# houzhijian/CONE

Measured on AMD Instinct MI355X. Metric: windows/sec + queries/sec, Ego4D-NLQ win_len=90 d=256 top-k=20, higher is better.
Workload: dtype f32

## Files before the change

### cone_amd/_lib.py

```python
from __future__ import annotations

import ctypes as C
import os

HERE = os.path.dirname(os.path.abspath(__file__))
LIB_PATH = os.path.join(HERE, "libcone_hip.so")

MAX_LAYERS = 8
MAX_PROJ = 3

c_float_p = C.c_void_p


class Linear(C.Structure):
    _fields_ = [("w", C.c_void_p), ("b", C.c_void_p)]


class LNorm(C.Structure):
    _fields_ = [("g", C.c_void_p), ("b", C.c_void_p)]


class Mha(C.Structure):
    _fields_ = [("in_proj_w", C.c_void_p), ("in_proj_b", C.c_void_p), ("out_proj", Linear)]

# ... 140 lines not shown
    "cone_criterion_forward": (C.c_int, [C.c_void_p, C.c_void_p, C.c_void_p, C.c_void_p, C.c_void_p, C.c_void_p, C.c_int,
                                         C.c_void_p, C.c_void_p, C.c_int, C.c_void_p, C.c_int, C.c_int, C.c_int,
                                         C.c_float, C.c_float, C.c_float, C.c_float, C.c_float, C.c_void_p, C.c_void_p,
                                         C.c_void_p, C.c_void_p]),
    "cone_adapter_nce": (C.c_int, [C.c_void_p, C.c_int, C.c_float, C.c_void_p, C.c_void_p]),
    "cone_prof_enable": (C.c_int, [C.c_int]),
    "cone_prof_collect": (C.c_int64, [C.c_void_p, C.c_int64]),
    "cone_eval_recall": (C.c_int, [C.c_void_p, C.c_void_p, C.c_void_p, C.c_int, C.c_int, C.c_void_p, C.c_int,
                                   C.c_void_p, C.c_int, C.c_int, C.c_void_p, C.c_void_p, C.c_void_p]),
    "cone_eval_window_recall": (C.c_int, [C.c_void_p, C.c_int, C.c_int, C.c_void_p, C.c_double, C.c_int, C.c_void_p,
                                          C.c_int, C.c_void_p, C.c_void_p]),
    "cone_model_set_option": (C.c_int, [C.c_void_p, C.c_char_p, C.c_int]),
    "cone_model_get_dims": (C.c_int, [C.c_void_p, C.POINTER(ModelDims)]),
    "cone_session_arena_bytes": (C.c_size_t, [C.c_void_p, C.c_int64, C.c_int]),
    "cone_session_workspace": (C.c_size_t, [C.c_void_p, C.c_int64, C.c_int]),
    "cone_session_index": (C.c_int, [C.c_void_p, C.c_void_p, C.c_int64, C.c_int, C.c_void_p, C.c_size_t, C.c_void_p, C.c_size_t,
                                     C.POINTER(Session), C.c_void_p]),
    "cone_session_query_layout": (C.c_int, [C.POINTER(C.c_int32), C.c_int, C.c_int, C.c_int64, C.c_int, C.c_int, C.c_int]
                                  + [C.c_void_p] * 8 + [C.c_void_p]),
    "cone_session_localize_workspace": (C.c_size_t, [C.c_void_p, C.POINTER(Session), C.POINTER(C.c_int32), C.c_int, C.c_int,
                                                     C.c_int, C.POINTER(SessionParams)]),
    "cone_session_localize": (C.c_int, [C.c_void_p, C.POINTER(Session), C.c_void_p, C.POINTER(C.c_int32), C.c_int, C.c_void_p,
                                        C.c_int, C.c_int, C.POINTER(SessionParams), C.c_void_p, C.c_void_p, C.c_void_p,
                                        C.c_void_p, C.c_size_t, C.c_void_p]),
    "cone_library_arena_bytes": (C.c_size_t, [C.c_void_p, C.c_int64, C.c_int]),
    "cone_library_open": (C.c_int, [C.c_void_p, C.c_int64, C.c_int, C.c_void_p, C.c_size_t, C.POINTER(Library)]),
    "cone_library_add_workspace": (C.c_size_t, [C.c_void_p, C.c_int64]),
    "cone_library_add": (C.c_int, [C.c_void_p, C.POINTER(Library), C.c_int64, C.c_void_p, C.c_int64, C.c_void_p, C.c_size_t,
                                   C.c_void_p]),
    "cone_library_query_layout": (C.c_int, [C.POINTER(C.c_int32)] * 3 + [C.c_int] * 5 + [C.c_void_p] * 8 + [C.c_void_p]),
    "cone_library_localize_workspace": (C.c_size_t, [C.c_void_p, C.POINTER(Library)] + [C.POINTER(C.c_int32)] * 3
                                        + [C.c_int, C.c_int, C.POINTER(SessionParams)]),
    "cone_library_localize": (C.c_int, [C.c_void_p, C.POINTER(Library), C.POINTER(C.c_int32), C.POINTER(C.c_int32), C.c_void_p,
                                        C.POINTER(C.c_int32), C.c_int, C.c_void_p, C.c_int, C.POINTER(SessionParams), C.c_void_p,
                                        C.c_void_p, C.c_void_p, C.c_size_t, C.c_void_p]),
    "cone_library_scan_workspace": (C.c_size_t, [C.POINTER(Library), C.c_int64, C.c_int64, C.c_int, C.c_int, C.c_int]),
    "cone_library_scan": (C.c_int, [C.c_void_p, C.POINTER(Library)] + [C.c_void_p] * 3 + [C.c_int64, C.c_int64, C.c_void_p, C.c_int,
                                    C.c_int, C.c_int, C.POINTER(SessionParams)] + [C.c_void_p] * 4 + [C.c_void_p, C.c_size_t,
                                                                                                    C.c_void_p]),
    "cone_library_localize_ranked_workspace": (C.c_size_t, [C.c_void_p, C.POINTER(Library)] + [C.POINTER(C.c_int32)] * 3
                                               + [C.c_int, C.c_int, C.POINTER(SessionParams)]),
    "cone_library_localize_ranked": (C.c_int, [C.c_void_p, C.POINTER(Library), C.POINTER(C.c_int32), C.POINTER(C.c_int32), C.c_void_p,
                                               C.POINTER(C.c_int32), C.c_int, C.c_void_p, C.c_int, C.POINTER(SessionParams),
                                               C.POINTER(C.c_int32), C.POINTER(C.c_int32), C.c_void_p, C.c_void_p, C.c_int, C.c_int64,
                                               C.c_int, C.c_void_p, C.c_void_p, C.c_void_p, C.c_size_t, C.c_void_p]),
    "cone_library_move_stage_bytes": (C.c_size_t, [C.POINTER(Library), C.c_int64]),
    "cone_library_move_rows": (C.c_int, [C.c_void_p, C.POINTER(Library), C.POINTER(Library)] + [C.c_void_p] * 3 + [C.c_int64] * 4
                               + [C.c_void_p, C.c_size_t, C.c_void_p]),
    "cone_library_budget_workspace": (C.c_size_t, [C.c_int, C.c_int64, C.c_int, C.c_int]),
    "cone_library_budget": (C.c_int, [C.c_void_p, C.c_int, C.c_int64, C.c_int, C.c_int] + [C.c_void_p] * 4
                            + [C.c_void_p, C.c_size_t, C.c_void_p]),
    "cone_library_localize_ragged_workspace": (C.c_size_t, [C.c_void_p, C.POINTER(Library)] + [C.POINTER(C.c_int32)] * 3
                                               + [C.c_int, C.POINTER(C.c_int32), C.POINTER(SessionParams), C.c_int]),
    "cone_library_localize_ragged": (C.c_int, [C.c_void_p, C.POINTER(Library), C.POINTER(C.c_int32), C.POINTER(C.c_int32), C.c_void_p,
                                               C.POINTER(C.c_int32), C.c_int, C.c_void_p, C.POINTER(C.c_int32),
                                               C.POINTER(SessionParams), C.POINTER(C.c_int32), C.POINTER(C.c_int32), C.c_void_p,
                                               C.c_void_p, C.c_int, C.c_int64, C.c_int, C.c_void_p, C.c_void_p, C.c_void_p, C.c_size_t,
                                               C.c_void_p]),
    "cone_corpus_fuse_nms": (C.c_int, [C.c_void_p] * 5 + [C.c_int, C.c_int, C.c_double, C.c_int, C.c_int] + [C.c_void_p] * 4),
    "cone_library_localize_candidates_workspace": (C.c_size_t, [C.c_void_p, C.POINTER(Library)] + [C.POINTER(C.c_int32)] * 3
                                                   + [C.c_int, C.POINTER(C.c_int32), C.POINTER(SessionParams), C.c_int]),
    "cone_library_localize_candidates": (C.c_int, [C.c_void_p, C.POINTER(Library), C.POINTER(C.c_int32), C.POINTER(C.c_int32),
                                                   C.c_void_p, C.POINTER(C.c_int32), C.c_int, C.c_void_p, C.POINTER(C.c_int32),
                                                   C.POINTER(SessionParams), C.POINTER(C.c_int32), C.POINTER(C.c_int32), C.c_void_p,
                                                   C.c_void_p, C.c_int, C.c_int64, C.c_int, C.c_void_p, C.c_void_p, C.c_size_t,
                                                   C.c_void_p]),
    "cone_watch_plan": (C.c_int, [C.c_void_p, C.c_void_p, C.c_int, C.c_int, C.c_void_p] + [C.c_int] * 4 + [C.c_void_p] * 8),
    "cone_watch_store": (C.c_int, [C.c_void_p] * 3 + [C.c_int] * 5 + [C.c_void_p] * 3),
    "cone_watch_pool_plan": (C.c_int, [C.c_void_p] * 9 + [C.c_int] * 7 + [C.c_void_p] * 8),
    "cone_watch_pool_store": (C.c_int, [C.c_void_p, C.c_void_p, C.c_int] + [C.c_void_p] * 4 + [C.c_int] * 5 + [C.c_void_p] * 3),
    "cone_library_shadow_bytes": (C.c_size_t, [C.POINTER(Library)]),
    "cone_library_shadow_open": (C.c_int, [C.POINTER(Library), C.c_void_p, C.c_size_t, C.POINTER(LibraryShadow)]),
    "cone_library_shadow_index": (C.c_int, [C.c_void_p, C.POINTER(Library), C.POINTER(LibraryShadow), C.c_int64, C.c_int64, C.c_void_p]),
    "cone_library_scan_certified_workspace": (C.c_size_t, [C.POINTER(Library), C.c_int64, C.c_int64, C.c_int64] + [C.c_int] * 4),
    "cone_library_scan_certified": (C.c_int, [C.c_void_p, C.POINTER(Library), C.POINTER(LibraryShadow)] + [C.c_void_p] * 4
                                    + [C.c_int64] * 3 + [C.c_void_p] + [C.c_int] * 4 + [C.POINTER(SessionParams)] + [C.c_void_p] * 3
                                    + [C.c_void_p, C.c_size_t, C.c_void_p]),
    "cone_test_gemm": (C.c_int, [C.c_void_p, C.c_void_p, C.c_int, C.c_void_p, C.c_void_p, C.c_void_p,
                                 C.c_void_p, C.c_void_p, C.c_void_p, C.c_void_p, C.c_void_p, C.c_int, C.c_int,
                                 C.c_int, C.c_int, C.c_void_p]),
    "cone_test_gemm_tall": (C.c_int, [C.c_void_p, C.c_void_p, C.c_int, C.c_void_p, C.c_void_p, C.c_void_p,
                                      C.c_void_p, C.c_void_p, C.c_void_p, C.c_void_p, C.c_void_p, C.c_int, C.c_int,
                                      C.c_int, C.c_int, C.c_int, C.c_int, C.c_void_p, C.c_int, C.c_void_p]),
    "cone_test_gemm_bf16_image_bytes": (C.c_size_t, [C.c_int, C.c_int]),
    "cone_test_gemm_bf16": (C.c_int, [C.c_void_p, C.c_void_p, C.c_int, C.c_void_p, C.c_void_p, C.c_void_p,
                                      C.c_void_p, C.c_void_p, C.c_void_p, C.c_void_p, C.c_void_p, C.c_int, C.c_int,
                                      C.c_int, C.c_int, C.c_void_p, C.c_int, C.c_int, C.c_void_p, C.c_void_p]),
    "cone_test_ffn": (C.c_int, [C.c_void_p] * 8 + [C.c_int, C.c_int, C.c_void_p]),
    "cone_test_proj_ffn": (C.c_int, [C.c_void_p] * 13 + [C.c_int, C.c_int, C.c_void_p]),
    "cone_test_tail_form": (C.c_int, [C.c_void_p] * 13 + [C.c_int, C.c_int] + [C.c_void_p] * 3 + [C.c_int, C.c_void_p, C.c_int, C.c_int,
                                                                               C.c_void_p, C.c_void_p]),
    "cone_test_proj_ffn_spread_scratch_bytes": (C.c_size_t, [C.c_int]),
    "cone_test_proj_ffn_spread": (C.c_int, [C.c_void_p] * 13 + [C.c_int, C.c_int, C.c_void_p, C.c_void_p]),
    "cone_test_ffn_split_image_bytes": (C.c_size_t, [C.c_int]),
    "cone_test_ffn_split": (C.c_int, [C.c_void_p] * 8 + [C.c_int, C.c_int, C.c_void_p, C.c_int, C.c_void_p]),
    "cone_test_rows_split_image_bytes": (C.c_size_t, [C.c_int]),
    "cone_test_rows_split": (C.c_int, [C.c_void_p] * 4 + [C.c_int, C.c_int, C.c_void_p, C.c_int, C.c_void_p]),
    "cone_test_proj_split_image_bytes": (C.c_size_t, []),
    "cone_test_proj_ffn_split": (C.c_int, [C.c_void_p] * 13 + [C.c_int, C.c_int, C.c_void_p, C.c_void_p, C.c_int, C.c_void_p]),
    "cone_test_enc_attn": (C.c_int, [C.c_int] + [C.c_void_p] * 9 + [C.c_int, C.c_int, C.c_int, C.c_void_p]),
    "cone_test_dec_cross": (C.c_int, [C.c_void_p] * 9 + [C.c_int] * 4 + [C.c_void_p, C.c_void_p]),
    "cone_test_dec_cross_slab_floats": (C.c_size_t, []),
    "cone_test_enc_attn_txt": (C.c_int, [C.c_int] + [C.c_void_p] * 10 + [C.c_int, C.c_int, C.c_int, C.c_void_p]),
    "cone_test_small_attn": (C.c_int, [C.c_void_p, C.c_int, C.c_void_p, C.c_int, C.c_void_p, C.c_int, C.c_void_p, C.c_int,
                                       C.c_void_p, C.c_int, C.c_int, C.c_int, C.c_void_p]),
    "cone_test_dec_cross_ex": (C.c_int, [C.c_void_p] * 10 + [C.c_int] * 4 + [C.c_void_p] * 4 + [C.c_int, C.c_void_p]),
    "cone_test_layernorm": (C.c_int, [C.c_void_p, C.c_void_p, C.c_void_p, C.c_void_p, C.c_int64, C.c_int,
                                      C.c_void_p]),
    "cone_test_gen_attn": (C.c_int, [C.c_void_p, C.c_int, C.c_void_p, C.c_int, C.c_void_p, C.c_int, C.c_void_p, C.c_int,
                                     C.c_void_p, C.c_void_p] + [C.c_int] * 5 + [C.c_void_p]),
    "cone_test_grid_limit_y": (C.c_int, []),
    "cone_test_scan_lengths": (C.c_int, [C.c_void_p, C.c_void_p, C.c_int, C.c_void_p, C.c_void_p]),
    "cone_test_compact_index": (C.c_int, [C.c_void_p, C.c_void_p, C.c_int, C.c_void_p, C.c_void_p, C.c_void_p, C.c_int,
                                          C.c_void_p, C.c_int, C.c_void_p]),
    "cone_test_pack_pos": (C.c_int, [C.c_void_p] * 11 + [C.c_int, C.c_int] + [C.c_void_p] * 4),
    "cone_test_gen_pack_pos": (C.c_int, [C.c_void_p] * 10 + [C.c_int] * 3 + [C.c_void_p] * 4),
    "cone_test_pack_l0": (C.c_int, [C.c_void_p] * 15 + [C.c_int, C.c_int, C.c_void_p]),
    "cone_test_row_index": (C.c_int, [C.c_void_p] * 6 + [C.c_int, C.c_int, C.c_void_p]),
    "cone_test_add_pos_rows": (C.c_int, [C.c_void_p] * 5 + [C.c_int, C.c_int] + [C.c_void_p] * 3),
    "cone_test_txt_pos_rows": (C.c_int, [C.c_void_p] * 3 + [C.c_int, C.c_int] + [C.c_void_p] * 3 + [C.c_int] + [C.c_void_p] * 3),
    "cone_test_gen_txt_pos_rows": (C.c_int, [C.c_void_p] * 3 + [C.c_int, C.c_int] + [C.c_void_p] * 3 + [C.c_int, C.c_void_p, C.c_int,
                                                                                                    C.c_void_p, C.c_void_p]),
    "cone_test_saliency": (C.c_int, [C.c_void_p] * 7 + [C.c_int, C.c_void_p, C.c_int, C.c_int, C.c_void_p]),
    "cone_test_gen_saliency": (C.c_int, [C.c_void_p] * 7 + [C.c_int, C.c_void_p, C.c_int, C.c_int, C.c_int, C.c_void_p]),
    "cone_test_rowdot": (C.c_int, [C.c_void_p, C.c_int, C.c_void_p, C.c_void_p, C.c_void_p, C.c_int, C.c_int64, C.c_int, C.c_int,
                                   C.c_void_p]),
    "cone_test_gen_rowdot": (C.c_int, [C.c_void_p, C.c_int, C.c_void_p, C.c_void_p, C.c_void_p, C.c_int, C.c_int64, C.c_int, C.c_int,
                                       C.c_int, C.c_void_p]),
    "cone_test_tile_rows": (C.c_int, [C.c_void_p, C.c_int, C.c_int64, C.c_void_p]),
    "cone_test_tile_rows2": (C.c_int, [C.c_void_p] * 4 + [C.c_int, C.c_int64, C.c_void_p]),
}
EXPORTS = tuple(_SIGNATURES)

_lib = None


class ConeHipError(RuntimeError):
    pass


def load():
    global _lib
    if _lib is not None:
        return _lib
    if not os.path.exists(LIB_PATH):
        raise ConeHipError(
            f"{LIB_PATH} is missing: build the HIP extension with `python -m cone_amd.build` "
            "(hipcc, gfx950). cone_amd has no CPU fallback.")
    import torch
    lib = C.CDLL(LIB_PATH)
    for name, (res, args) in _SIGNATURES.items():
        fn = getattr(lib, name)
        fn.restype = res
        fn.argtypes = args
    if lib.cone_abi_version() != 8:
        raise ConeHipError("libcone_hip.so ABI version mismatch; rebuild")
    _lib = lib
    return lib


_pylists = None


def pylists():
    global _pylists
    if _pylists is None:
# ... 42 lines not shown
```

### cone_amd/build.py

```python
from __future__ import annotations

import os
import subprocess
import sys
from concurrent.futures import ThreadPoolExecutor

HERE = os.path.dirname(os.path.abspath(__file__))
CSRC = os.path.join(HERE, "csrc")
OBJ = os.path.join(CSRC, "_obj")
LIB = os.path.join(HERE, "libcone_hip.so")
PYLISTS = os.path.join(HERE, "_cone_pylists.so")
SOURCES = ["api.hip", "gemm.hip", "rowops.hip", "attention.hip", "window_ops.hip", "prefilter.hip",
           "postproc.hip", "prof.hip", "dec_cross.hip", "metrics.hip", "ffn.hip", "criterion.hip", "dec_cross_mfma.hip", "ffn_split.hip", "ffn_wide.hip",
           "general.hip", "ffn_bf16.hip", "gemm_bf16.hip", "gemm_tall.hip", "session.hip", "library_move.hip",
           "library_budget.hip", "library_corpus.hip", "library_watch.hip", "library_watch_pool.hip"]
FLAGS = ["-O3", "--offload-arch=gfx950", "-fPIC", "-std=c++17", "-Wall", "-Wno-unused-function"]
NO_CONTRACT = {"window_ops.hip", "postproc.hip", "metrics.hip", "criterion.hip", "general.hip", "library_corpus.hip"}


def _deps_mtime():
    hdrs = [os.path.join(CSRC, f) for f in os.listdir(CSRC) if f.endswith(".h")]
    hdrs += [os.path.join(HERE, "..", "include", "cone_hip.h"), __file__]
    return max(os.path.getmtime(h) for h in hdrs)


def _compile(src):
    obj = os.path.join(OBJ, src.replace(".hip", ".o"))
    stamp = obj + ".flags"
    path = os.path.join(CSRC, src)
    extra = ["-ffp-contract=off"] if src in NO_CONTRACT else []
    extra += os.environ.get("CONE_HIPCC_FLAGS", "").split()
    flags = " ".join([*FLAGS, *extra])
    try:
        with open(stamp) as f:
            same_flags = f.read() == flags
    except OSError:
        same_flags = False
    if same_flags and os.path.exists(obj) and os.path.getmtime(obj) >= max(os.path.getmtime(path), _deps_mtime()):
        return obj
    cmd = ["hipcc", *FLAGS, *extra, "-c", path, "-o", obj]
    r = subprocess.run(cmd, capture_output=True, text=True)
    if r.returncode != 0:
        raise RuntimeError(f"hipcc failed for {src}:\n{r.stdout}\n{r.stderr}")
    with open(stamp, "w") as f:
        f.write(flags)
    if r.stderr.strip():
        sys.stderr.write(r.stderr)
    return obj


def build(force: bool = False) -> str:
    os.makedirs(OBJ, exist_ok=True)
    if force:
        for f in os.listdir(OBJ):
            os.remove(os.path.join(OBJ, f))
    with ThreadPoolExecutor(max_workers=4) as ex:
        objs = list(ex.map(_compile, SOURCES))
    if (not os.path.exists(LIB)) or any(os.path.getmtime(o) > os.path.getmtime(LIB) for o in objs):
        r = subprocess.run(["hipcc", "--offload-arch=gfx950", "-shared", "-fPIC", "-o", LIB, *objs],
                           capture_output=True, text=True)
        if r.returncode != 0:
            raise RuntimeError(f"link failed:\n{r.stdout}\n{r.stderr}")
    try:
        build_pylists()
    except (RuntimeError, OSError) as e:
        try:
            if os.path.exists(PYLISTS) and os.path.getmtime(PYLISTS) < os.path.getmtime(os.path.join(CSRC, "pylists.c")):
                os.remove(PYLISTS)
        except OSError:
            pass
        sys.stderr.write(f"cone_amd.build: _cone_pylists.so not built ({str(e).splitlines()[0]}); "
                         "submission lists will be built by the Python loop\n")
    return LIB


def build_pylists() -> str:
    import sysconfig
    src = os.path.join(CSRC, "pylists.c")
    if os.path.exists(PYLISTS) and os.path.getmtime(PYLISTS) >= max(os.path.getmtime(src), os.path.getmtime(__file__)):
        return PYLISTS
    r = subprocess.run(["gcc", "-O2", "-shared", "-fPIC", "-Wall", "-I", sysconfig.get_paths()["include"], src, "-o", PYLISTS],
                       capture_output=True, text=True)
    if r.returncode != 0:
        raise RuntimeError(f"gcc failed for pylists.c:\n{r.stdout}\n{r.stderr}")
    return PYLISTS


if __name__ == "__main__":
    print(build(force="--force" in sys.argv))
```

### cone_amd/csrc/api.hip

```cpp
#include <stdarg.h>
#include <string.h>

#include <vector>

#include "common.h"
#include "gemm_tall.h"
#include "rows_chain.h"

namespace cone {

static thread_local char g_err[512] = "";
void set_error(const char* fmt, ...) {
    va_list ap;
    va_start(ap, fmt);
    vsnprintf(g_err, sizeof(g_err), fmt, ap);
    va_end(ap);
}

struct Linear { const float* w = nullptr; const float* b = nullptr; };
struct LNorm { const float* g = nullptr; const float* b = nullptr; };
struct Mha { const float* in_w = nullptr; const float* in_b = nullptr; Linear out; };
struct EncLayer { Mha sa; Linear l1, l2; LNorm n1, n2; };
struct DecLayer { Mha sa, ca; Linear l1, l2; LNorm n1, n2, n3; };

}

struct cone_model {
    int d, heads, ff, n_enc, n_dec, nq, n_proj, dt, dv, dvm, has_adapter;
    float* arena = nullptr;
    cone::LNorm vproj_ln[CONE_MAX_PROJ], tproj_ln[CONE_MAX_PROJ];
    cone::Linear vproj[CONE_MAX_PROJ], tproj[CONE_MAX_PROJ];
    cone::EncLayer enc[CONE_MAX_LAYERS];
    cone::DecLayer dec[CONE_MAX_LAYERS];
    cone::LNorm dec_norm;
    const float* query_embed = nullptr;
    cone::Linear class_embed, span[3], saliency, adapter[2];
    const float* dim_t = nullptr;
    const float* txt_pos_emb = nullptr; int txt_pos_rows = 0; cone::LNorm txt_pos_ln;
    int pre_norm = 0; cone::LNorm enc_norm;
    cone::Linear dec_k, dec_v;
    const float* dec_vT[CONE_MAX_LAYERS] = {};
    float* dec0_tgt1 = nullptr; float* dec0_dq = nullptr; float* dec0_scratch = nullptr;
    float* dec_sa_tab[CONE_MAX_LAYERS] = {}; float* dec_ca_tab[CONE_MAX_LAYERS] = {};
    float* tab_arena = nullptr; const float* tab_pos_rows = nullptr; const float* tab_pos_qk = nullptr; int tab_max_v_l = 0;
    int opt_dec_fold = 2;
    int opt_dec0_const = 1;
    int opt_l0_gather = 1;
    int opt_pos_tables = 1;
    int opt_gemm = 0;
    int opt_gemm_tall_min = -1;
    cone::TailWeights enc_tail[CONE_MAX_LAYERS] = {}, dec_tail[CONE_MAX_LAYERS] = {};
    char* split_img = nullptr; char* bf16_img = nullptr;
    int opt_qkv_fused = 1;
    int opt_split_bf16 = 0;
    int opt_bf16 = 0;
    int opt_res_gather = 1;
    int opt_spread = 1;
    int opt_chain = 1;
    int opt_ffn_fused = 2;
    int gen_native = 0;
    int opt_general = 0;
    int opt_general_bf16 = 0;
    char* gen_bf16_img = nullptr;
    struct GenImage { const float* W; const void* img; };
    std::vector<GenImage> gen_bf16_images;
    int opt_max_tokens = CONE_MAX_WINDOW_TOKENS;
    bool long_windows() const { return opt_max_tokens > CONE_MAX_WINDOW_TOKENS; }
    bool general() const { return gen_native || opt_general || long_windows(); }
};

namespace cone {

struct ArenaBuilder {
    struct Item { const float* src; size_t n; const float** dst; };
    std::vector<Item> items;
    size_t total = 0;
    void add(const float* src, size_t n, const float** dst) {
        items.push_back({src, n, dst});
        total += align_up(n, 64);
    }
};

static int dec0_constants(cone_model* m, hipStream_t s);
static int build_pos_tables(const cone_model* m, int max_v_l, float* pos_rows, float* pos_qk, hipStream_t s);
static int64_t pos_table_rows(int max_v_l) { return (int64_t)max_v_l * (max_v_l + 1) / 2 + 1; }

static void free_model(cone_model* m) {
    if (m->arena) (void)hipFree(m->arena);
    if (m->split_img) (void)hipFree(m->split_img);
    if (m->bf16_img) (void)hipFree(m->bf16_img);
    if (m->gen_bf16_img) (void)hipFree(m->gen_bf16_img);
    if (m->tab_arena) (void)hipFree(m->tab_arena);
    delete m;
}

static const TailMode* const TAIL_MODES[TAIL_IMG_MODES] = {&TAIL_MODE_SPLIT, &TAIL_MODE_BF16};
static int build_tail_images(cone_model* m, int mode, char** img) {
    const TailMode& k = *TAIL_MODES[mode];
    const size_t per = k.proj_image_bytes() + k.ffn_image_bytes(m->ff), qkv = k.rows_image_bytes(768);
    if (hipMalloc((void**)img, per * (size_t)(m->n_enc + m->n_dec) + qkv * (size_t)m->n_enc) != hipSuccess) {
        set_error("model_create: building the split-bf16 / bf16 weight images failed");
        return CONE_E_HIP;
    }
    char* ip = *img;
    for (int l = 0; l < m->n_enc; ++l, ip += qkv) {
        if (int rc = k.pack(m->enc_tail[l].Wq, nullptr, 768, ip, nullptr)) return rc;
        m->enc_tail[l].img[mode].qkv = ip;
    }
    for (int i = 0; i < m->n_enc + m->n_dec; ++i, ip += per) {
        TailWeights& t = i < m->n_enc ? m->enc_tail[i] : m->dec_tail[i - m->n_enc];
        if (int rc = k.pack(t.Wo, nullptr, 256, ip, nullptr)) return rc;
        if (int rc = k.pack(t.W1, t.W2, m->ff, ip + k.proj_image_bytes(), nullptr)) return rc;
        t.img[mode].wo = ip; t.img[mode].ffn = ip + k.proj_image_bytes();
    }
    return 0;
}

static int build_model(const cone_weights* w, cone_model** out) {
    CONE_REQUIRE(w && out, "model_create: null argument");
    const bool shipped = w->hidden_dim == 256 && w->nheads == 8;
    CONE_REQUIRE(shipped || gen_shape_supported(w->hidden_dim, w->nheads),
                 "model_create: unsupported model shape hidden_dim=%d nheads=%d -- supported: hidden_dim a multiple of 64 in "
                 "[64, 512] with head_dim = hidden_dim / nheads in {16, 32, 64} (256 / 8, every shipped CONE configuration, runs "
                 "the fused kernels; other shapes the general path); also required: dim_feedforward a multiple of 128, "
                 "num_queries <= 16, feature dims multiples of 32 up to 1024, at most 256 tokens (clips + words) per window (up to 1024 with "
                 "option max_window_tokens)",
                 w->hidden_dim, w->nheads);
    CONE_REQUIRE(w->dim_ff % 128 == 0 && w->dim_ff >= 128, "model_create: dim_feedforward=%d must be a multiple of 128", w->dim_ff);
    CONE_REQUIRE(w->enc_layers >= 1 && w->enc_layers <= CONE_MAX_LAYERS && w->dec_layers >= 1 &&
                     w->dec_layers <= CONE_MAX_LAYERS, "model_create: layer counts out of range");
    CONE_REQUIRE(w->num_queries >= 1 && w->num_queries <= 16, "model_create: num_queries=%d not in [1,16]", w->num_queries);
    CONE_REQUIRE(w->n_input_proj >= 1 && w->n_input_proj <= CONE_MAX_PROJ, "model_create: n_input_proj out of range");
    CONE_REQUIRE(w->t_dim % 32 == 0 && w->v_dim % 32 == 0 && w->v_motion_dim % 32 == 0 && w->t_dim <= 1024 && w->v_dim <= 1024 &&
                     w->v_motion_dim <= 1024 && w->t_dim > 0 && w->v_dim > 0 && w->v_motion_dim > 0,
                 "model_create: feature dims must be multiples of 32 and <= 1024 (t=%d v_appear=%d v_motion=%d)", w->t_dim,
                 w->v_dim, w->v_motion_dim);
    cone_model* m = new cone_model();
    m->d = w->hidden_dim; m->heads = w->nheads; m->gen_native = !shipped; m->ff = w->dim_ff; m->n_enc = w->enc_layers; m->n_dec = w->dec_layers;
    m->nq = w->num_queries; m->n_proj = w->n_input_proj; m->dt = w->t_dim; m->dv = w->v_dim; m->dvm = w->v_motion_dim;
    m->has_adapter = w->has_adapter;
    const size_t d = m->d, ff = m->ff;
    ArenaBuilder ab;
    auto lin = [&](const cone_linear_w& s, size_t nout, size_t nin, Linear& dst) {
        ab.add(s.w, nout * nin, &dst.w);
        ab.add(s.b, nout, &dst.b);
    };
    auto ln = [&](const cone_ln_w& s, size_t n, LNorm& dst) { ab.add(s.g, n, &dst.g); ab.add(s.b, n, &dst.b); };
    auto mha = [&](const cone_mha_w& s, Mha& dst) {
        ab.add(s.in_proj_w, 3 * d * d, &dst.in_w);
        ab.add(s.in_proj_b, 3 * d, &dst.in_b);
        lin(s.out_proj, d, d, dst.out);
    };
    for (int i = 0; i < m->n_proj; ++i) {
        ln(w->vid_proj_ln[i], i == 0 ? m->dvm : d, m->vproj_ln[i]);
        lin(w->vid_proj[i], d, i == 0 ? m->dvm : d, m->vproj[i]);
        ln(w->txt_proj_ln[i], i == 0 ? m->dt : d, m->tproj_ln[i]);
        lin(w->txt_proj[i], d, i == 0 ? m->dt : d, m->tproj[i]);
    }
    for (int i = 0; i < m->n_enc; ++i) {
        mha(w->enc[i].self_attn, m->enc[i].sa);
        lin(w->enc[i].linear1, ff, d, m->enc[i].l1);
        lin(w->enc[i].linear2, d, ff, m->enc[i].l2);
        ln(w->enc[i].norm1, d, m->enc[i].n1);
        ln(w->enc[i].norm2, d, m->enc[i].n2);
    }
    for (int i = 0; i < m->n_dec; ++i) {
        mha(w->dec[i].self_attn, m->dec[i].sa);
        mha(w->dec[i].cross_attn, m->dec[i].ca);
        lin(w->dec[i].linear1, ff, d, m->dec[i].l1);
        lin(w->dec[i].linear2, d, ff, m->dec[i].l2);
        ln(w->dec[i].norm1, d, m->dec[i].n1);
        ln(w->dec[i].norm2, d, m->dec[i].n2);
        ln(w->dec[i].norm3, d, m->dec[i].n3);
    }
    ln(w->dec_norm, d, m->dec_norm);
    ab.add(w->query_embed, (size_t)m->nq * d, &m->query_embed);
    lin(w->class_embed, 2, d, m->class_embed);
    lin(w->span_embed[0], d, d, m->span[0]);
    lin(w->span_embed[1], d, d, m->span[1]);
    lin(w->span_embed[2], 2, d, m->span[2]);
    lin(w->saliency_proj, 1, d, m->saliency);
    if (m->has_adapter) {
        lin(w->adapter[0], d, m->dv, m->adapter[0]);
        lin(w->adapter[1], m->dv, d, m->adapter[1]);
    }
    ab.add(w->pos_dim_t, d, &m->dim_t);
    if (w->txt_pos_embed) {
        if (w->txt_pos_rows < 1 || w->txt_pos_rows > 4096 || !w->txt_pos_ln.g || !w->txt_pos_ln.b) {
            free_model(m);
            set_error("model_create: txt_pos_embed needs txt_pos_rows in [1, 4096] (got %d) and its LayerNorm", w->txt_pos_rows);
            return CONE_E_INVALID;
        }
        m->txt_pos_rows = w->txt_pos_rows;
        ab.add(w->txt_pos_embed, (size_t)w->txt_pos_rows * d, &m->txt_pos_emb);
        ln(w->txt_pos_ln, d, m->txt_pos_ln);
    }
    if (w->pre_norm) {
// ... 17 lines not shown
        return CONE_E_HIP;
    }
    size_t cur = 0;
    for (auto& it : ab.items) {
        e = hipMemcpy(m->arena + cur, it.src, it.n * sizeof(float), hipMemcpyDefault);
        if (e != hipSuccess) {
            free_model(m);
            set_error("model_create: weight copy failed: %s", hipGetErrorString(e));
            return CONE_E_HIP;
        }
        *it.dst = m->arena + cur;
        cur += align_up(it.n, 64);
    }
    float* kw = m->arena + cur; cur += align_up((size_t)m->n_dec * d * d, 64);
    float* kb = m->arena + cur; cur += align_up((size_t)m->n_dec * d, 64);
    float* vw = m->arena + cur; cur += align_up((size_t)m->n_dec * d * d, 64);
    float* vb = m->arena + cur; cur += align_up((size_t)m->n_dec * d, 64);
    for (int i = 0; i < m->n_dec; ++i) {
        const float* iw = m->dec[i].ca.in_w;
        const float* ib = m->dec[i].ca.in_b;
        (void)hipMemcpy(kw + (size_t)i * d * d, iw + d * d, d * d * sizeof(float), hipMemcpyDeviceToDevice);
        (void)hipMemcpy(kb + (size_t)i * d, ib + d, d * sizeof(float), hipMemcpyDeviceToDevice);
        (void)hipMemcpy(vw + (size_t)i * d * d, iw + 2 * d * d, d * d * sizeof(float), hipMemcpyDeviceToDevice);
        e = hipMemcpy(vb + (size_t)i * d, ib + 2 * d, d * sizeof(float), hipMemcpyDeviceToDevice);
    }
    if (e != hipSuccess || hipDeviceSynchronize() != hipSuccess) {
        free_model(m);
        set_error("model_create: stacking decoder K/V weights failed");
        return CONE_E_HIP;
    }
    m->dec_k = {kw, kb};
    m->dec_v = {vw, vb};
    {
        std::vector<float> h(d * d), ht(d * d);
        for (int i = 0; i < m->n_dec; ++i) {
            float* dst = m->arena + cur; cur += d * d;
            e = hipMemcpy(h.data(), m->dec[i].ca.in_w + 2 * d * d, d * d * sizeof(float), hipMemcpyDeviceToHost);
            for (size_t o = 0; o < d; ++o)
                for (size_t c = 0; c < d; ++c) ht[c * d + o] = h[o * d + c];
            if (e == hipSuccess) e = hipMemcpy(dst, ht.data(), d * d * sizeof(float), hipMemcpyHostToDevice);
            if (e != hipSuccess) {
                free_model(m);
                set_error("model_create: transposing decoder V weights failed: %s", hipGetErrorString(e));
                return CONE_E_HIP;
            }
            m->dec_vT[i] = dst;
        }
    }
    m->dec0_tgt1 = m->arena + cur; cur += align_up((size_t)m->nq * d, 64);
    m->dec0_dq = m->arena + cur; cur += align_up((size_t)m->nq * d, 64);
    m->dec0_scratch = m->arena + cur; cur += align_up((size_t)m->nq * (d + 3 * d + d), 64);
    for (int i = 0; i < m->n_dec; ++i) {
        m->dec_sa_tab[i] = m->arena + cur; cur += align_up((size_t)m->nq * 3 * d, 64);
        m->dec_ca_tab[i] = m->arena + cur; cur += align_up((size_t)m->nq * d, 64);
    }
    auto tail = [](const Linear& o, const Linear& l1, const Linear& l2, const LNorm& in, const LNorm& outn) {
        TailWeights t{};
        t.Wo = o.w; t.bo = o.b; t.W1 = l1.w; t.b1 = l1.b; t.W2 = l2.w; t.b2 = l2.b;
        t.in_g = in.g; t.in_b = in.b; t.out_g = outn.g; t.out_b = outn.b;
        return t;
    };
    for (int l = 0; l < m->n_enc; ++l) {
        const EncLayer& el = m->enc[l];
        const LNorm& nxt = l + 1 < m->n_enc ? m->enc[l + 1].n1 : m->enc_norm;
        m->enc_tail[l] = m->pre_norm ? tail(el.sa.out, el.l1, el.l2, el.n2, nxt) : tail(el.sa.out, el.l1, el.l2, el.n1, el.n2);
        m->enc_tail[l].Wq = el.sa.in_w; m->enc_tail[l].qb = el.sa.in_b;
    }
    for (int l = 0; l < m->n_dec; ++l) {
        const DecLayer& dl = m->dec[l];
        m->dec_tail[l] = m->pre_norm ? tail(dl.ca.out, dl.l1, dl.l2, dl.n3, m->dec_norm) : tail(dl.ca.out, dl.l1, dl.l2, dl.n2, dl.n3);
    }
    if (!m->gen_native && TAIL_MODES[TAIL_IMG_SPLIT]->ffn_supported(m->ff)) {
        int rc = build_tail_images(m, TAIL_IMG_SPLIT, &m->split_img);
        if (rc == 0) rc = build_tail_images(m, TAIL_IMG_BF16, &m->bf16_img);
        if (rc == 0 && hipDeviceSynchronize() != hipSuccess) {
            set_error("model_create: building the split-bf16 / bf16 weight images failed");
            rc = CONE_E_HIP;
        }
        if (rc != 0) {
            free_model(m);
            return CONE_E_HIP;
        }
    }
    if (dec0_constants(m, nullptr) != 0 || hipDeviceSynchronize() != hipSuccess) {
        free_model(m);
        return CONE_E_HIP;
    }
    if (!m->gen_native) {
        const int tab_l = (w->table_max_v_l >= 1 && w->table_max_v_l <= CONE_TABLE_MAX_V_L) ? w->table_max_v_l : CONE_TABLE_MAX_V_L;
        const size_t rows = (size_t)pos_table_rows(tab_l);
        e = hipMalloc((void**)&m->tab_arena, rows * (256 + 512 * (size_t)m->n_enc) * sizeof(float));
        int rc = e == hipSuccess ? 0 : CONE_E_HIP;
        if (rc == 0) rc = build_pos_tables(m, tab_l, m->tab_arena, m->tab_arena + rows * 256, nullptr);
        if (rc != 0 || hipDeviceSynchronize() != hipSuccess) {
            if (e != hipSuccess) set_error("model_create: hipMalloc of the position tables failed: %s", hipGetErrorString(e));
            free_model(m);
            return CONE_E_HIP;
        }
        m->tab_pos_rows = m->tab_arena; m->tab_pos_qk = m->tab_arena + rows * 256; m->tab_max_v_l = tab_l;
    }
    *out = m;
    return 0;
}

struct Carver {
    char* base; size_t cap, cur = 0; bool ok = true;
    Carver(void* p, size_t n) : base((char*)p), cap(n) {}
    template <typename T> T* take(size_t n) {
        const size_t bytes = align_up(n * sizeof(T), 256);
        T* r = (T*)(base + cur);
        cur += bytes;
        if (cur > cap) ok = false;
        return r;
    }
};

static GemmArgs G(const cone_model* m, const float* A, int lda, const float* W, int ldw, const float* bias, float* C,
                  int ldc, int M, const int* M_dev, int N, int K, int flags = 0) {
    GemmArgs g{};
    g.A = A; g.lda = lda; g.W = W; g.ldw = ldw; g.bias = bias; g.C = C; g.ldc = ldc;
    g.M = M; g.M_dev = M_dev; g.N = N; g.K = K; g.flags = flags;
    g.variant = m ? m->opt_gemm | ((m->opt_gemm_tall_min + 1) << GEMM_TALL_MIN_SHIFT) : GEMM_AUTO;
    if (m && !m->opt_spread) g.flags |= GEMM_NO_SPREAD;
    return g;
}

#define RUN(expr) do { int _rc = (expr); if (_rc) return _rc; } while (0)

static int dec0_constants(cone_model* m, hipStream_t s) {
    const int nq = m->nq, d = m->d;
    float* TGT = m->dec0_scratch;
    float* QKV = TGT + (size_t)nq * 256;
    float* DATT = QKV + (size_t)nq * 768;
    CONE_CHECK_HIP(hipMemsetAsync(TGT, 0, (size_t)nq * d * sizeof(float), s));
    for (int l = 0; l < m->n_dec; ++l) {
        const DecLayer& dl = m->dec[l];
        RUN(launch_gemm(G(m, m->query_embed, d, dl.sa.in_w, d, dl.sa.in_b, m->dec_sa_tab[l], 3 * d, nq, nullptr, 2 * d, d), s));
        RUN(launch_gemm(G(m, TGT, d, dl.sa.in_w + 2 * d * d, d, dl.sa.in_b + 2 * d, m->dec_sa_tab[l] + 2 * d, 3 * d, nq, nullptr, d, d), s));
        RUN(launch_gemm(G(m, m->query_embed, d, dl.ca.in_w, d, dl.ca.in_b, m->dec_ca_tab[l], d, nq, nullptr, d, d), s));
    }
    if (m->gen_native) return 0;
    const DecLayer& d0 = m->dec[0];
    GemmArgs g = G(m, TGT, 256, d0.sa.in_w, 256, nullptr, QKV, 768, nq, nullptr, 768, 256, EPI_RESIDUAL);
    g.R = m->dec_sa_tab[0]; g.ldr = 768; g.r_mod = nq;
    RUN(launch_gemm(g, s));
    RUN(launch_small_attn(QKV, 768, QKV + 256, 768, QKV + 512, 768, DATT, 256, nullptr, 1, nq, nq, s));
    g = G(m, DATT, 256, d0.sa.out.w, 256, d0.sa.out.b, m->dec0_tgt1, 256, nq, nullptr, 256, 256, EPI_RESIDUAL | EPI_LN);
    g.R = TGT; g.ldr = 256; g.ln_g = d0.n1.g; g.ln_b = d0.n1.b;
    RUN(launch_gemm(g, s));
    g = G(m, m->dec0_tgt1, 256, d0.ca.in_w, 256, nullptr, m->dec0_dq, 256, nq, nullptr, 256, 256, EPI_RESIDUAL);
    g.R = m->dec_ca_tab[0]; g.ldr = 256; g.r_mod = nq;
    RUN(launch_gemm(g, s));
    return 0;
}

static int build_pos_tables(const cone_model* m, int max_v_l, float* pos_rows, float* pos_qk, hipStream_t s) {
    const int64_t rows = pos_table_rows(max_v_l);
    if (m->d != 256) {
        const int d = m->d;
        RUN(launch_gen_pos_rows(m->dim_t, max_v_l, d, pos_rows, s));
        CONE_CHECK_HIP(hipMemsetAsync(pos_rows + (size_t)(rows - 1) * d, 0, d * sizeof(float), s));
        for (int l = 0; l < m->n_enc; ++l)
            RUN(launch_gemm(G(m, pos_rows, d, m->enc[l].sa.in_w, d, nullptr, pos_qk + (size_t)l * rows * 2 * d, 2 * d, (int)rows,
                              nullptr, 2 * d, d), s));
        return 0;
    }
    RUN(launch_pos_rows(m->dim_t, max_v_l, pos_rows, s));
    CONE_CHECK_HIP(hipMemsetAsync(pos_rows + (size_t)(rows - 1) * 256, 0, 256 * sizeof(float), s));
    for (int l = 0; l < m->n_enc; ++l)
        RUN(launch_gemm(G(m, pos_rows, 256, m->enc[l].sa.in_w, 256, nullptr, pos_qk + (size_t)l * rows * 512, 512,
                          (int)rows, nullptr, 512, 256), s));
    return 0;
}

static int encoder_qkv(const cone_model* m, int l, const float* X, float* QKV, int M, const int* M_dev, hipStream_t s,
                       bool split_ok) {
    const TailWeights& t = m->enc_tail[l];
    const int d = m->d;
    const int mode = m->opt_bf16 && m->bf16_img && !m->general()               ? TAIL_IMG_BF16
                     : split_ok && l > 0 && m->opt_split_bf16 && m->split_img ? TAIL_IMG_SPLIT
                                                                               : -1;
    if (mode >= 0) return TAIL_MODES[mode]->rows256(X, 256, t.img[mode].qkv, t.qb, QKV, 768, M, M_dev, 768, s);
    return launch_gemm(G(m, X, d, t.Wq, d, t.qb, QKV, 3 * d, M, M_dev, 3 * d, d), s);
}

static int layer0_rows(const cone_model* m, const float* rows, int n, const int* n_dev, float* qkv, float* tmp, hipStream_t s) {
    const float* a = rows;
    const int d = m->d;
    if (m->pre_norm) {
        RUN(launch_layernorm(rows, d, m->enc[0].n1.g, m->enc[0].n1.b, tmp, d, n, n_dev, d, s));
        a = tmp;
    }
    return encoder_qkv(m, 0, a, qkv, n, n_dev, s, false);
}

static size_t project_ws_bytes(const cone_model* m, int which, int64_t n) {
    const size_t din = which == 0 ? m->dvm : m->dt;
    return align_up(n * din * 4, 256) + (m->d == 256 ? 2 : 3) * align_up(n * m->d * 4, 256);
}
static int project_tokens(const cone_model* m, int which, const float* x, int64_t n, float* out, void* ws,
                          size_t ws_bytes, hipStream_t s, const int* src_row = nullptr, const int* n_dev = nullptr) {
    CONE_REQUIRE(n < (1ll << 31), "project: too many rows");
    const int din = which == 0 ? m->dvm : m->dt;
    const LNorm* lns = which == 0 ? m->vproj_ln : m->tproj_ln;
    const Linear* lin = which == 0 ? m->vproj : m->tproj;
    const int d = m->d;
// ... 187 lines not shown
    const int nd = m->n_dec, Lmax = c.Lv_max + c.Lq_max;
    const float* XP = p.dec_tab ? nullptr : f.XP;
    const float* pos = p.dec_tab ? p.l0.pos_rows : nullptr;
    if (p.cross[l] == CROSS_SMALL)
        return launch_small_attn(f.DQ, 256, f.KD + l * 256, 256 * nd, f.VD + l * 256, 256 * nd, f.DATT, 256, f.off, c.B, m->nq, Lmax, s);
    if (p.cross[l] == CROSS_VALU)
        return launch_dec_cross(f.DQ, XP, MEM, pos, c.vlen, f.off, dl.ca.in_w + 256 * 256, m->dec_vT[l], dl.ca.in_b + 512, f.DATT, c.B,
                                m->nq, Lmax, s);
    const bool ride = l == 0 && p.sal_ride;
    if (ride) CONE_CHECK_HIP(hipMemsetAsync(c.saliency, 0, (size_t)c.B * c.Lv_max * sizeof(float), s));
    return launch_dec_cross_mfma(f.DQ, XP, MEM, pos, c.vlen, f.off, dl.ca.in_w + 256 * 256, m->dec_vT[l], dl.ca.in_b + 512, f.DATT,
                                 c.B, m->nq, Lmax, l == 0 && p.slabs ? f.QKS : nullptr, s, p.cross[l], ride ? m->saliency.w : nullptr,
                                 ride ? m->saliency.b : nullptr, ride ? c.saliency : nullptr, ride ? c.Lv_max : 0);
}
static AttnSrc table_attn_src(const FwdCall& c, const cone_layer0& l0, int l) {
    const size_t rows = (size_t)pos_table_rows(l0.max_v_l);
    AttnSrc src{};
    src.vlen = c.vlen; src.pos_zero_row = (int)rows - 1;
    src.pos_qk = l0.pos_qk + (size_t)l * rows * 512;
    if (l0.txt_pos_qk) { src.txt_pos_qk = l0.txt_pos_qk + (size_t)l * l0.n_txt * 512; src.trow0 = c.trow0; }
    return src;
}

static int forward_packed_prenorm(const cone_model* m, const FwdCall& c, const FwdPlan& p, FwdBuffers& f, hipStream_t s) {
    const int B = c.B, Lmax = c.Lv_max + c.Lq_max, Mmax = B * Lmax, T = B * m->nq, nd = m->n_dec, ff = m->ff;
    const int* Mdev = f.off + B;
    RUN(launch_scan_lengths(c.vlen, c.qlen, B, f.off, s));
    RUN(launch_pack_pos(c.vproj, c.vrow0, c.vlen, c.tproj, c.trow0, c.qlen, f.off, m->dim_t, f.X, f.POS, f.XP, B, Lmax, s,
                        m->txt_pos_emb, m->txt_pos_ln.g, m->txt_pos_ln.b));
    GemmArgs g;
    for (int l = 0; l < m->n_enc; ++l) {
        const EncLayer& e = m->enc[l];
        RUN(launch_layernorm(f.X, 256, e.n1.g, e.n1.b, f.X1, 256, Mmax, Mdev, 256, s));
        float* QK = f.QKV; float* V = f.QKV + (size_t)Mmax * 512;
        g = G(m, f.X1, 256, e.sa.in_w, 256, e.sa.in_b, QK, 512, Mmax, Mdev, 512, 256);
        g.A2 = f.POS; g.lda2 = 256;
        RUN(launch_gemm(g, s));
        RUN(launch_gemm(G(m, f.X1, 256, e.sa.in_w + 512 * 256, 256, e.sa.in_b + 512, V, 256, Mmax, Mdev, 256, 256), s));
        AttnSrc src{};
        src.Q = QK; src.K = QK + 256; src.V = V; src.ldq = src.ldk = 512; src.ldv = 256;
        RUN(launch_enc_attn(ATTN_PACKED, src, f.ATT, f.off, B, Lmax, s));
        g = G(m, f.ATT, 256, e.sa.out.w, 256, e.sa.out.b, f.X, 256, Mmax, Mdev, 256, 256, EPI_RESIDUAL);
        g.R = f.X; g.ldr = 256;
        RUN(launch_gemm(g, s));
        RUN(launch_layernorm(f.X, 256, e.n2.g, e.n2.b, f.X1, 256, Mmax, Mdev, 256, s));
        RUN(launch_gemm(G(m, f.X1, 256, e.l1.w, 256, e.l1.b, f.H, ff, Mmax, Mdev, ff, 256, EPI_RELU), s));
        g = G(m, f.H, ff, e.l2.w, ff, e.l2.b, f.X, 256, Mmax, Mdev, 256, ff, EPI_RESIDUAL);
        g.R = f.X; g.ldr = 256;
        RUN(launch_gemm(g, s));
    }
    RUN(launch_layernorm(f.X, 256, m->enc_norm.g, m->enc_norm.b, f.X1, 256, Mmax, Mdev, 256, s));
    const float* MEM = f.X1;
    g = G(m, MEM, 256, m->dec_k.w, 256, m->dec_k.b, f.KD, 256 * nd, Mmax, Mdev, 256 * nd, 256);
    g.A2 = f.POS; g.lda2 = 256;
    RUN(launch_gemm(g, s));
    RUN(launch_gemm(G(m, MEM, 256, m->dec_v.w, 256, m->dec_v.b, f.VD, 256 * nd, Mmax, Mdev, 256 * nd, 256), s));
    CONE_CHECK_HIP(hipMemsetAsync(f.TGT, 0, (size_t)T * 256 * sizeof(float), s));
    for (int l = 0; l < nd; ++l) {
        const DecLayer& dl = m->dec[l];
        RUN(dec_layer_front(m, f, l, B, true, s));
        RUN(dec_cross_attn(m, c, p, f, l, MEM, s));
        g = G(m, f.DATT, 256, dl.ca.out.w, 256, dl.ca.out.b, f.TGT, 256, T, nullptr, 256, 256, EPI_RESIDUAL);
        g.R = f.TGT; g.ldr = 256;
        RUN(launch_gemm(g, s));
        RUN(launch_layernorm(f.TGT, 256, dl.n3.g, dl.n3.b, f.TGT1, 256, T, nullptr, 256, s));
        RUN(launch_gemm(G(m, f.TGT1, 256, dl.l1.w, 256, dl.l1.b, f.DH, ff, T, nullptr, ff, 256, EPI_RELU), s));
        g = G(m, f.DH, ff, dl.l2.w, ff, dl.l2.b, f.TGT, 256, T, nullptr, 256, ff, EPI_RESIDUAL);
        g.R = f.TGT; g.ldr = 256;
        RUN(launch_gemm(g, s));
        RUN(launch_layernorm(f.TGT, 256, m->dec_norm.g, m->dec_norm.b, f.HS + (size_t)l * T * 256, 256, T, nullptr, 256, s));
    }
    return heads_and_taps(m, c, HeadBufs{f.HS, f.S1, f.S2, f.LG, f.SP, f.off}, MEM, false, s);
}

static int launch_layer_tail(const cone_model* m, const FwdBuffers& f, TailArgs t, hipStream_t s, bool* rode = nullptr) {
    bool no_ride;
    if (!rode) rode = &no_ride;
    const TailWeights* next = t.next;
    const int ff = t.ff;
    const bool bf16 = m->opt_bf16 && m->bf16_img, split = m->opt_split_bf16 && m->split_img;
    const bool spread = m->opt_spread && f.SPR && ffn_spread_supported(t.M, ff);
    t.next = nullptr;
    t.scratch = f.SPR;
    *rode = false;
    if (t.pre) {
        if (bf16) return TAIL_MODES[TAIL_IMG_BF16]->proj_ffn_prenorm(t, s);
        if (spread) return launch_proj_ffn_spread(t, s);
        if (m->opt_spread && (t.M + 15) / 16 <= FFN_WIDE_GROUPS && ffn_wide_supported(ff)) return launch_proj_ffn_prenorm_wide(t, s);
        return launch_proj_ffn_prenorm(t, s);
    }
    const bool block_fused = !t.C2 && m->opt_ffn_fused && ffn_fused_supported(ff);
    if (block_fused && m->opt_ffn_fused >= 2) {
        if (bf16 || split) {
            const TailMode& k = *TAIL_MODES[bf16 ? TAIL_IMG_BF16 : TAIL_IMG_SPLIT];
            *rode = next && m->opt_qkv_fused && k.qkv_fits(ff, t.n_qkv);
            if (*rode) t.next = next;
            return k.proj_ffn(t, s);
        }
        *rode = next && m->opt_qkv_fused >= 2 && ffn_fused_qkv_fits(ff, t.n_qkv);
        if (*rode) t.next = next;
        else if (spread) return launch_proj_ffn_spread(t, s);
        return launch_proj_ffn_fused(t, s);
    }
    const TailWeights& w = *t.w;
    GemmArgs g = G(m, t.A, t.lda, w.Wo, 256, w.bo, t.X1, 256, t.M, t.M_dev, 256, 256, EPI_RESIDUAL | EPI_LN);
    g.R = t.R; g.ldr = t.ldr; g.ln_g = w.in_g; g.ln_b = w.in_b;
    RUN(launch_gemm(g, s));
    if (block_fused)
        return launch_ffn_fused(t.X1, 256, w.W1, w.b1, w.W2, w.b2, w.out_g, w.out_b, t.OUT, t.ldo, t.M, t.M_dev, ff, s);
    RUN(launch_gemm(G(m, t.X1, 256, w.W1, 256, w.b1, t.H, ff, t.M, t.M_dev, ff, 256, EPI_RELU), s));
    g = G(m, t.H, ff, w.W2, ff, w.b2, t.OUT, t.ldo, t.M, t.M_dev, 256, ff, EPI_RESIDUAL | EPI_LN);
    g.R = t.X1; g.ldr = 256; g.ln_g = w.out_g; g.ln_b = w.out_b;
    g.C2 = t.C2; g.ADD = t.ADD;
    return launch_gemm(g, s);
}
static TailArgs tail_args(const TailWeights* w, const float* A, const float* R, float* OUT, int M, const int* M_dev, int ff) {
    TailArgs t{};
    t.A = A; t.lda = 256; t.R = R; t.ldr = 256; t.w = w; t.OUT = OUT; t.ldo = 256; t.M = M; t.M_dev = M_dev; t.ff = ff;
    return t;
}

struct GenBuffers {
    int* off;
    float *X, *X1, *T1, *POS, *QKV, *ATT, *H, *KD, *VD;
    float *TGT, *TGT1, *TGT2, *DQK, *DATT, *DQ, *DH, *HS, *S1, *S2, *LG, *SP;
};
static void carve_gen(const cone_model* m, Carver& c, int B, int Lmax, GenBuffers& f) {
    const size_t M = (size_t)B * Lmax, T = (size_t)B * m->nq, nd = m->n_dec, d = m->d;
    f.off = c.take<int>(B + 1);
    f.X = c.take<float>(M * d); f.X1 = c.take<float>(M * d); f.T1 = c.take<float>(M * d); f.POS = c.take<float>(M * d);
    f.QKV = c.take<float>(M * 3 * d); f.ATT = c.take<float>(M * d); f.H = c.take<float>(M * m->ff);
    f.KD = c.take<float>(M * d * nd); f.VD = c.take<float>(M * d * nd);
    f.TGT = c.take<float>(T * d); f.TGT1 = c.take<float>(T * d); f.TGT2 = c.take<float>(T * d);
    f.DQK = c.take<float>(T * 3 * d); f.DATT = c.take<float>(T * d); f.DQ = c.take<float>(T * d); f.DH = c.take<float>(T * m->ff);
    f.HS = c.take<float>(nd * T * d); f.S1 = c.take<float>(nd * T * d); f.S2 = c.take<float>(nd * T * d);
    f.LG = c.take<float>(nd * T * 2); f.SP = c.take<float>(nd * T * 2);
}
static size_t fwd_ws_bytes(const cone_model* m, int B, int Lmax, const FwdPlan& p) {
    Carver c(nullptr, ~(size_t)0);
    FwdBuffers f;
    GenBuffers g;
    if (p.body == BODY_GENERAL) carve_gen(m, c, B, Lmax, g);
    else carve_fwd(m, c, B, Lmax, p, f);
    return c.cur;
}

static int forward_general(const cone_model* m, const FwdCall& call, void* ws, size_t ws_bytes, hipStream_t s) {
    const int d = m->d, hd = m->d / m->heads, nh = m->heads, B = call.B;
    const int Lmax = call.Lv_max + call.Lq_max, Mmax = B * Lmax, T = B * m->nq, nd = m->n_dec, ff = m->ff, nq = m->nq;
    const bool pre = m->pre_norm != 0;
    const int kcap = m->long_windows() ? m->opt_max_tokens : Lmax;
    Carver c(ws, ws_bytes);
    GenBuffers f;
    carve_gen(m, c, B, Lmax, f);
    if (!c.ok) { set_error("forward: workspace too small (%zu < %zu)", ws_bytes, c.cur); return CONE_E_WORKSPACE; }
    const int* Mdev = f.off + B;
    RUN(launch_scan_lengths(call.vlen, call.qlen, B, f.off, s));
    RUN(launch_gen_pack_pos(call.vproj, call.vrow0, call.vlen, call.tproj, call.trow0, call.qlen, f.off, m->dim_t, f.X, f.POS, d, B,
                            Lmax, s, m->txt_pos_emb, m->txt_pos_ln.g, m->txt_pos_ln.b));
    GemmArgs g;
    auto gemm = [&](const GemmArgs& a) {
        if (!m->opt_general_bf16) return launch_gemm(a, s);
        const void* img = nullptr;
        for (const cone_model::GenImage& gi : m->gen_bf16_images)
            if (gi.W == a.W) { img = gi.img; break; }
        CONE_REQUIRE(img, "forward: general_bf16 is set but a weight has no bf16 image");
// ... 495 lines not shown
}
extern "C" int cone_clip_matching(const cone_model* m, const float* cls, const float* vid, const int32_t* vid_len,
                                  int Lv_pad, const float* spans, int B, float* match, void* ws, size_t ws_bytes,
                                  void* stream) {
    CONE_REQUIRE(m && ws, "clip_matching: null argument");
    if (B <= 0) return 0;
    hipStream_t s = (hipStream_t)stream;
    Carver c(ws, ws_bytes);
    int* vrow0 = c.take<int>(B);
    int* padl = c.take<int>(B);
    if (!c.ok) { set_error("clip_matching: workspace too small"); return CONE_E_WORKSPACE; }
    hipLaunchKernelGGL(iota_fill_kernel, dim3((B + 255) / 256), dim3(256), 0, s, vrow0, padl, B, Lv_pad, Lv_pad);
    CONE_LAUNCH_CHECK();
    return cone_clip_matching_gathered(m, cls, nullptr, vid, vrow0, vid_len, padl, spans, B, match,
                                       (char*)ws + c.cur, ws_bytes - c.cur, stream);
}

static int build_general_bf16_images(cone_model* m) {
    struct Item { const float* W; int N, K; };
    std::vector<Item> items;
    const int d = m->d, ff = m->ff, nd = m->n_dec;
    for (int l = 0; l < m->n_enc; ++l) {
        const EncLayer& e = m->enc[l];
        items.push_back({e.sa.in_w, 2 * d, d});
        items.push_back({e.sa.in_w + (size_t)2 * d * d, d, d});
        items.push_back({e.sa.out.w, d, d});
        items.push_back({e.l1.w, ff, d});
        items.push_back({e.l2.w, d, ff});
    }
    items.push_back({m->dec_k.w, d * nd, d});
    items.push_back({m->dec_v.w, d * nd, d});
    for (int l = 0; l < nd; ++l) {
        const DecLayer& dl = m->dec[l];
        items.push_back({dl.sa.in_w, 3 * d, d});
        items.push_back({dl.sa.out.w, d, d});
        items.push_back({dl.ca.in_w, d, d});
        items.push_back({dl.ca.out.w, d, d});
        items.push_back({dl.l1.w, ff, d});
        items.push_back({dl.l2.w, d, ff});
    }
    size_t total = 0;
    for (const Item& it : items) {
        CONE_REQUIRE(gemm_bf16_image_bytes(it.N, it.K), "set_option: general_bf16: a %d x %d weight has no bf16 image form", it.N, it.K);
        total += gemm_bf16_image_bytes(it.N, it.K);
    }
    char* base = nullptr;
    hipError_t e = hipMalloc((void**)&base, total);
    if (e != hipSuccess) {
        set_error("set_option: general_bf16: hipMalloc of %zu bytes of weight images failed: %s", total, hipGetErrorString(e));
        return CONE_E_HIP;
    }
    std::vector<cone_model::GenImage> images;
    char* ip = base;
    int rc = 0;
    for (const Item& it : items) {
        rc = launch_gemm_bf16_pack(it.W, it.K, it.N, it.K, ip, nullptr);
        if (rc) break;
        images.push_back({it.W, ip});
        ip += gemm_bf16_image_bytes(it.N, it.K);
    }
    if (rc == 0 && hipDeviceSynchronize() != hipSuccess) {
        set_error("set_option: general_bf16: building the weight images failed");
        rc = CONE_E_HIP;
    }
    if (rc) { (void)hipFree(base); return rc; }
    m->gen_bf16_img = base;
    m->gen_bf16_images.swap(images);
    return 0;
}

struct OptionRow { const char* name; int cone_model::*field; int lo, hi; bool is_switch; };
static const OptionRow OPTION_ROWS[] = {
    {"dec_fold", &cone_model::opt_dec_fold, 0, 5, false},
    {"l0_gather", &cone_model::opt_l0_gather, 0, 1, true},
    {"dec0_const", &cone_model::opt_dec0_const, 0, 1, true},
    {"pos_tables", &cone_model::opt_pos_tables, 0, 1, true},
    {"ffn_fused", &cone_model::opt_ffn_fused, 0, 2, false},
    {"qkv_fused", &cone_model::opt_qkv_fused, 0, 2, false},
    {"general_shape", &cone_model::opt_general, 0, 1, true},
    {"res_gather", &cone_model::opt_res_gather, 0, 1, true},
    {"rows_chain", &cone_model::opt_chain, 0, 1, true},
    {"ffn_spread", &cone_model::opt_spread, 0, 1, true},
    {"gemm_tall_min_rows", &cone_model::opt_gemm_tall_min, -1, GEMM_TALL_MIN_MAX, false},
};
extern "C" int cone_model_set_option(cone_model* m, const char* name, int value) {
    CONE_REQUIRE(m && name, "set_option: null argument");
    for (const OptionRow& o : OPTION_ROWS) {
        if (strcmp(name, o.name)) continue;
        CONE_REQUIRE(o.is_switch || (value >= o.lo && value <= o.hi), "set_option: %s %d not in [%d, %d]", name, value, o.lo, o.hi);
        m->*o.field = o.is_switch ? value != 0 : value;
        return 0;
    }
    if (!strcmp(name, "max_window_tokens")) {
        CONE_REQUIRE(value >= CONE_MAX_WINDOW_TOKENS && value <= CONE_MAX_LONG_WINDOW_TOKENS,
                     "set_option: max_window_tokens %d not in [%d, %d]", value, CONE_MAX_WINDOW_TOKENS, CONE_MAX_LONG_WINDOW_TOKENS);
        CONE_REQUIRE(value == CONE_MAX_WINDOW_TOKENS || !(m->opt_bf16 || m->opt_split_bf16),
                     "set_option: max_window_tokens %d while bf16 / split_bf16 = 1: windows beyond %d tokens run in exact fp32 "
                     "only (set the mode to 0 first)", value, CONE_MAX_WINDOW_TOKENS);
        m->opt_max_tokens = value;
        return 0;
    }
    const bool split = !strcmp(name, "split_bf16");
    if (split || !strcmp(name, "bf16")) {
        const char* other = split ? "bf16" : "split_bf16";
        CONE_REQUIRE(value == 0 || !m->long_windows(),
                     "set_option: %s on a handle with max_window_tokens = %d: windows beyond %d tokens run the general path, "
                     "exact fp32 only", name, m->opt_max_tokens, CONE_MAX_WINDOW_TOKENS);
        CONE_REQUIRE(value == 0 || (split ? m->split_img : m->bf16_img),
                     "set_option: %s needs hidden_dim 256 with 8 heads and dim_feedforward %% 32 == 0 "
                     "(<= 2048); this handle is hidden_dim %d with %d heads, dim_feedforward %d", name, m->d, m->heads, m->ff);
        CONE_REQUIRE(value == 0 || !(split ? m->opt_bf16 : m->opt_split_bf16),
                     "set_option: %s = 1 while %s = 1: the two modes exclude each other (set %s = 0 first)", name, other, other);
        (split ? m->opt_split_bf16 : m->opt_bf16) = value != 0;
        return 0;
    }
    if (!strcmp(name, "general_bf16")) {
        if (value == 0) { m->opt_general_bf16 = 0; return 0; }
        CONE_REQUIRE(m->general(),
                     "set_option: general_bf16 applies to the general path only; this handle runs the fused path: use bf16 "
                     "(or general_shape = 1 / max_window_tokens first)");
        CONE_REQUIRE(m->ff % 32 == 0 && m->ff <= 2048,
                     "set_option: general_bf16 needs dim_feedforward %% 32 == 0 and <= 2048; this handle has dim_feedforward %d", m->ff);
        if (!m->gen_bf16_img)
            if (int rc = build_general_bf16_images(m)) return rc;
        m->opt_general_bf16 = 1;
        return 0;
    }
    if (!strcmp(name, "gemm")) {
        CONE_REQUIRE(value >= GEMM_AUTO && value <= GEMM_TALL, "set_option: gemm tile family %d not in [0, 4]", value);
        m->opt_gemm = value;
        if (dec0_constants(m, nullptr) != 0 || hipDeviceSynchronize() != hipSuccess) return CONE_E_HIP;
        return 0;
    }
    cone::set_error("set_option: unknown option '%s'", name);
    return CONE_E_INVALID;
}

extern "C" int cone_model_get_dims(const cone_model* m, cone_model_dims* out) {
    CONE_REQUIRE(m && out, "model_get_dims: null argument");
    out->hidden_dim = m->d; out->num_queries = m->nq; out->enc_layers = m->n_enc;
    out->t_dim = m->dt; out->v_dim = m->dv; out->v_motion_dim = m->dvm;
    out->txt_pos = m->txt_pos_emb != nullptr;
    out->long_windows = m->long_windows();
    return 0;
}

extern "C" int cone_test_gemm(const float* A, const float* A2, int a2_mod, const float* W, const float* bias,
                              const float* R, const float* ln_g, const float* ln_b, float* C, float* C2,
                              const float* ADD, int M, int N, int K, int flags, void* stream) {
    GemmArgs g = G(nullptr, A, K, W, K, bias, C, N, M, nullptr, N, K, flags & 0xff);
    g.variant = (flags >> 8) & 3;
    g.A2 = A2; g.lda2 = K; g.a2_mod = a2_mod; g.R = R; g.ldr = N; g.ln_g = ln_g; g.ln_b = ln_b;
    g.C2 = C2; g.ADD = ADD;
    return launch_gemm(g, (hipStream_t)stream);
}
extern "C" int cone_test_gemm_tall(const float* A, const float* A2, int a2_mod, const float* W, const float* bias,
                                   const float* R, const float* ln_g, const float* ln_b, float* C, float* C2,
                                   const float* ADD, int M, int N, int K, int flags, int lda, int ldc, const int32_t* M_dev,
                                   int n_cu, void* stream) {
    GemmArgs g = G(nullptr, A, lda ? lda : K, W, K, bias, C, ldc ? ldc : N, M, M_dev, N, K, flags & 0xff);
    g.variant = ((flags >> 8) & 7) | (((flags >> 11) & 1) << GEMM_TALL_MIN_SHIFT);
    g.A2 = A2; g.lda2 = K; g.a2_mod = a2_mod; g.R = R; g.ldr = ldc ? ldc : N; g.ln_g = ln_g; g.ln_b = ln_b;
    g.C2 = C2; g.ADD = ADD;
    CONE_REQUIRE(n_cu >= 0, "gemm tall hook: negative CU count");
    return n_cu > 0 ? launch_gemm_tall(g, n_cu, (hipStream_t)stream) : launch_gemm(g, (hipStream_t)stream);
}
extern "C" size_t cone_test_gemm_bf16_image_bytes(int N, int K) { return gemm_bf16_image_bytes(N, K); }
extern "C" int cone_test_gemm_bf16(const float* A, const float* A2, int a2_mod, const float* W, const float* bias,
                                   const float* R, const float* ln_g, const float* ln_b, float* C, float* C2,
                                   const float* ADD, int M, int N, int K, int flags, void* img, int ldc, int r_mod,
                                   const int32_t* M_dev, void* stream) {
    GemmArgs g = G(nullptr, A, K, W, K, bias, C, ldc ? ldc : N, M, M_dev, N, K, flags & 0xff);
    g.A2 = A2; g.lda2 = K; g.a2_mod = a2_mod; g.R = R; g.ldr = N; g.r_mod = r_mod; g.ln_g = ln_g; g.ln_b = ln_b;
    g.C2 = C2; g.ADD = ADD;
    if (int rc = launch_gemm_bf16_pack(W, K, N, K, img, (hipStream_t)stream)) return rc;
    return launch_gemm_bf16(g, img, (hipStream_t)stream);
}
extern "C" int cone_test_ffn(const float* X, const float* W1, const float* b1, const float* W2, const float* b2,
                             const float* ln_g, const float* ln_b, float* OUT, int M, int ff, void* stream) {
    return launch_ffn_fused(X, 256, W1, b1, W2, b2, ln_g, ln_b, OUT, 256, M, nullptr, ff, (hipStream_t)stream);
}
static TailArgs test_tail(TailWeights* w, const float* A, const float* Wo, const float* bo, const float* R, const float* pg,
                          const float* pb, const float* W1, const float* b1, const float* W2, const float* b2, const float* ln_g,
                          const float* ln_b, float* OUT, int M, int ff) {
    *w = TailWeights{};
    w->Wo = Wo; w->bo = bo; w->W1 = W1; w->b1 = b1; w->W2 = W2; w->b2 = b2; w->in_g = pg; w->in_b = pb; w->out_g = ln_g; w->out_b = ln_b;
    return tail_args(w, A, R, OUT, M, nullptr, ff);
}
extern "C" int cone_test_proj_ffn(const float* A, const float* Wo, const float* bo, const float* R, const float* pg,
                                  const float* pb, const float* W1, const float* b1, const float* W2, const float* b2,
                                  const float* ln_g, const float* ln_b, float* OUT, int M, int ff, void* stream) {
    TailWeights w;
    return launch_proj_ffn_fused(test_tail(&w, A, Wo, bo, R, pg, pb, W1, b1, W2, b2, ln_g, ln_b, OUT, M, ff), (hipStream_t)stream);
}
extern "C" size_t cone_test_proj_ffn_spread_scratch_bytes(int ff) { return ffn_spread_scratch_floats(ff) * sizeof(float); }
extern "C" int cone_test_proj_ffn_spread(const float* A, const float* Wo, const float* bo, const float* R, const float* pg,
                                         const float* pb, const float* W1, const float* b1, const float* W2, const float* b2,
                                         const float* ln_g, const float* ln_b, float* OUT, int M, int ff, void* scratch,
                                         void* stream) {
    TailWeights w;
    TailArgs t = test_tail(&w, A, Wo, bo, R, pg, pb, W1, b1, W2, b2, ln_g, ln_b, OUT, M, ff);
    t.scratch = (float*)scratch;
    return launch_proj_ffn_spread(t, (hipStream_t)stream);
}
extern "C" int cone_test_tail_form(const float* A, const float* Wo, const float* bo, const float* R, const float* pg,
                                   const float* pb, const float* W1, const float* b1, const float* W2, const float* b2,
                                   const float* ln_g, const float* ln_b, float* OUT, int M, int ff, const int32_t* r_idx,
                                   const float* R2, const int32_t* M_dev, int pre, float* OUT2, int form, int n_cu, void* scratch,
                                   void* stream) {
    TailWeights w;
    TailArgs t = test_tail(&w, A, Wo, bo, R, pg, pb, W1, b1, W2, b2, ln_g, ln_b, OUT, M, ff);
    t.r_idx = r_idx; t.R2 = R2; t.M_dev = M_dev; t.pre = pre != 0; t.OUT2 = OUT2; t.ldo2 = 256; t.scratch = (float*)scratch;
    return launch_tail_f32_form(t, form, n_cu, (hipStream_t)stream);
}
static int test_tail_mode(int pack, bool* do_pack) {
    const bool single = pack & CONE_TEST_SINGLE_PIECE;
    *do_pack = single ? pack & CONE_TEST_PACK : pack;
    return single ? TAIL_IMG_BF16 : TAIL_IMG_SPLIT;
}
extern "C" size_t cone_test_ffn_split_image_bytes(int ff) {
    const TailMode& k = *TAIL_MODES[TAIL_IMG_SPLIT];
    return k.ffn_supported(ff) ? k.ffn_image_bytes(ff) : 0;
}
extern "C" int cone_test_ffn_split(const float* X, const float* W1, const float* b1, const float* W2, const float* b2,
                                   const float* ln_g, const float* ln_b, float* OUT, int M, int ff, void* img, int pack,
                                   void* stream) {
    bool do_pack;
    const TailMode& k = *TAIL_MODES[test_tail_mode(pack, &do_pack)];
    if (do_pack) {
        const int rc = k.pack(W1, W2, ff, img, (hipStream_t)stream);
        if (rc) return rc;
    }
    return k.ffn(X, 256, img, b1, b2, ln_g, ln_b, OUT, 256, M, nullptr, ff, (hipStream_t)stream);
}
extern "C" size_t cone_test_rows_split_image_bytes(int N) {
    const TailMode& k = *TAIL_MODES[TAIL_IMG_SPLIT];
    return k.rows_supported(N) ? k.rows_image_bytes(N) : 0;
}
extern "C" int cone_test_rows_split(const float* X, const float* W, const float* bias, float* C, int M, int N, void* img,
                                    int pack, void* stream) {
    bool do_pack;
    const TailMode& k = *TAIL_MODES[test_tail_mode(pack, &do_pack)];
    if (do_pack) {
        const int rc = k.pack(W, nullptr, N, img, (hipStream_t)stream);
        if (rc) return rc;
    }
    return k.rows256(X, 256, img, bias, C, N, M, nullptr, N, (hipStream_t)stream);
}
extern "C" size_t cone_test_proj_split_image_bytes(void) { return TAIL_MODES[TAIL_IMG_SPLIT]->proj_image_bytes(); }
extern "C" int cone_test_proj_ffn_split(const float* A, const float* Wo, const float* bo, const float* R, const float* pg,
                                        const float* pb, const float* W1, const float* b1, const float* W2,
                                        const float* b2, const float* ln_g, const float* ln_b, float* OUT, int M, int ff,
                                        void* img, void* wo_img, int pack, void* stream) {
    bool do_pack;
    const int mode = test_tail_mode(pack, &do_pack);
    const TailMode& k = *TAIL_MODES[mode];
    if (do_pack) {
        int rc = k.pack(W1, W2, ff, img, (hipStream_t)stream);
        if (rc) return rc;
        rc = k.pack(Wo, nullptr, 256, wo_img, (hipStream_t)stream);
        if (rc) return rc;
    }
    TailWeights w;
    const TailArgs t = test_tail(&w, A, Wo, bo, R, pg, pb, W1, b1, W2, b2, ln_g, ln_b, OUT, M, ff);
    w.img[mode] = TailImages{wo_img, img, nullptr};
    return k.proj_ffn(t, (hipStream_t)stream);
}
extern "C" int cone_test_enc_attn(int mode, const float* QKV, const float* qkv_vid, const float* qkv_txt,
                                  const float* pos_qk, const int32_t* vrow0, const int32_t* vlen, const int32_t* trow0,
                                  const int32_t* off, float* OUT, int B, int Lmax, int pos_zero_row, void* stream) {
    AttnSrc a{};
    a.pos_zero_row = pos_zero_row;
    a.Q = QKV; a.K = QKV ? QKV + 256 : nullptr; a.V = QKV ? QKV + 512 : nullptr; a.ldq = a.ldk = a.ldv = 768;
    a.qkv_vid = qkv_vid; a.qkv_txt = qkv_txt; a.pos_qk = pos_qk; a.vrow0 = vrow0; a.vlen = vlen; a.trow0 = trow0;
    a.form = (mode >> 8) & 3;
    return launch_enc_attn(mode & 0xff, a, OUT, off, B, Lmax, (hipStream_t)stream);
}
extern "C" int cone_test_dec_cross(const float* DQ, const float* X, const float* pos_rows, const int32_t* vlen,
                                   const int32_t* off, const float* Wk, const float* WvT, const float* bv, float* OUT,
                                   int B, int nq, int Lmax, int variant, float* qk_slabs, void* stream) {
    if (variant == 1)
        return launch_dec_cross(DQ, nullptr, X, pos_rows, vlen, off, Wk, WvT, bv, OUT, B, nq, Lmax, (hipStream_t)stream);
    return launch_dec_cross_mfma(DQ, nullptr, X, pos_rows, vlen, off, Wk, WvT, bv, OUT, B, nq, Lmax, qk_slabs,
                                 (hipStream_t)stream, variant);
}
extern "C" size_t cone_test_dec_cross_slab_floats(void) { return dec_cross_mfma_slab_floats(); }
extern "C" int cone_test_enc_attn_txt(int mode, const float* QKV, const float* qkv_vid, const float* qkv_txt,
                                      const float* pos_qk, const float* txt_pos_qk, const int32_t* vrow0,
                                      const int32_t* vlen, const int32_t* trow0, const int32_t* off, float* OUT, int B,
                                      int Lmax, int pos_zero_row, void* stream) {
    AttnSrc a{};
    a.pos_zero_row = pos_zero_row;
    a.Q = QKV; a.K = QKV ? QKV + 256 : nullptr; a.V = QKV ? QKV + 512 : nullptr; a.ldq = a.ldk = a.ldv = 768;
    a.qkv_vid = qkv_vid; a.qkv_txt = qkv_txt; a.pos_qk = pos_qk; a.vrow0 = vrow0; a.vlen = vlen; a.trow0 = trow0;
    a.txt_pos_qk = txt_pos_qk;
    a.form = (mode >> 8) & 3;
// ... 99 lines not shown
```

### cone_amd/csrc/common.h

```cpp
#pragma once
#include <hip/hip_runtime.h>
#include <stdint.h>
#include <stdio.h>

#include <mutex>

#include "../../include/cone_hip.h"

namespace cone {

void set_error(const char* fmt, ...);

#define CONE_CHECK_HIP(expr)                                                                  \
    do {                                                                                      \
        hipError_t _e = (expr);                                                               \
        if (_e != hipSuccess) {                                                               \
            cone::set_error("%s failed: %s (%s:%d)", #expr, hipGetErrorString(_e), __FILE__,  \
                            __LINE__);                                                        \
            return CONE_E_HIP;                                                                \
        }                                                                                     \
    } while (0)

#define CONE_REQUIRE(cond, ...)          \
    do {                                 \
// ... 1 lines not shown
            cone::set_error(__VA_ARGS__); \
            return CONE_E_INVALID;       \
        }                                \
    } while (0)

#define CONE_LAUNCH_CHECK() CONE_CHECK_HIP(hipGetLastError())

static inline size_t align_up(size_t x, size_t a) { return (x + a - 1) / a * a; }

constexpr int CONE_MAX_DEVICES = 64;
struct DeviceOnce {
    std::mutex mu;
    bool done[CONE_MAX_DEVICES] = {};
    hipError_t rc[CONE_MAX_DEVICES] = {};
    int n_cu[CONE_MAX_DEVICES] = {};
};
template <typename F>
static inline hipError_t device_once(DeviceOnce& st, F&& setup, int* n_cu = nullptr) {
    int dev = 0;
    hipError_t e = hipGetDevice(&dev);
    if (e != hipSuccess) return e;
    if (dev < 0 || dev >= CONE_MAX_DEVICES) return hipErrorInvalidDevice;
    std::lock_guard<std::mutex> lk(st.mu);
    if (!st.done[dev]) {
        st.rc[dev] = setup();
        if (st.rc[dev] == hipSuccess)
            st.rc[dev] = hipDeviceGetAttribute(&st.n_cu[dev], hipDeviceAttributeMultiprocessorCount, dev);
        st.done[dev] = true;
    }
    if (n_cu) *n_cu = st.n_cu[dev];
    return st.rc[dev];
}

typedef float f32x16 __attribute__((ext_vector_type(16)));
typedef float f32x4 __attribute__((ext_vector_type(4)));

#ifdef __HIPCC__
__device__ __forceinline__ float wave_sum(float v) {
#pragma unroll
    for (int o = 32; o >= 1; o >>= 1) v += __shfl_xor(v, o, 64);
    return v;
}
__device__ __forceinline__ float wave_max(float v) {
#pragma unroll
    for (int o = 32; o >= 1; o >>= 1) v = fmaxf(v, __shfl_xor(v, o, 64));
    return v;
}
__device__ __forceinline__ float half_sum(float v) {
#pragma unroll
    for (int o = 16; o >= 1; o >>= 1) v += __shfl_xor(v, o, 64);
    return v;
}
__device__ __forceinline__ int acc_row(int r, int lane) { return (r & 3) + 8 * (r >> 2) + 4 * (lane >> 5); }
#endif

enum ProfKind { PK_GEMM_128x128 = 0, PK_GEMM_128x128_A2 = 1, PK_GEMM_64x256 = 2, PK_ENC_ATTN = 3, PK_FRAME_SCORE = 4,
                PK_GEMM_ROWS = 5, PK_GEMM_ROWS16 = 6, PK_DEC_CROSS = 7, PK_FFN_FUSED = 8, PK_FFN_PROJ = 9,
                PK_FFN_WIDE = 10, PK_FFN_PROJ_WIDE = 11, PK_FFN_FUSED_NW4 = 12, PK_FFN_PROJ_NW4 = 13, PK_GEMM_ROWS_SMALL = 14 };
bool prof_enabled();
struct ProfScope {
    ProfScope(int kind, int64_t a, int64_t b, int64_t c, const int* a_dev, hipStream_t s, int64_t a_off = 0);
    ~ProfScope();
    int idx_; hipStream_t s_; bool counted_;
};

enum { EPI_RELU = 1, EPI_RESIDUAL = 2, EPI_LN = 4,
       GEMM_NO_SPREAD = 8 };

struct GemmArgs {
    const float* A; int lda;
    const float* A2; int lda2; int a2_mod;
    const float* W; int ldw;
    const float* bias;
    const float* R; int ldr;
    int r_mod;
    const float* ln_g; const float* ln_b;
    float* C; int ldc;
    float* C2; const float* ADD;
    int M; const int* M_dev;
    int m_off;
    int N, K;
    int flags;
    int variant;
};
enum { GEMM_AUTO = 0, GEMM_SQUARE = 1, GEMM_ROWS4 = 2, GEMM_ROWS8 = 3 };
int launch_gemm(const GemmArgs& a, hipStream_t s);

size_t gemm_bf16_image_bytes(int N, int K);
int launch_gemm_bf16_pack(const float* W, int ldw, int N, int K, void* img, hipStream_t s);
int launch_gemm_bf16(const GemmArgs& a, const void* w_img, hipStream_t s);

enum { TAIL_IMG_SPLIT = 0, TAIL_IMG_BF16 = 1, TAIL_IMG_MODES = 2 };
struct TailImages { const void* wo; const void* ffn; const void* qkv; };
struct TailWeights {
    const float *Wo, *bo;
    const float *W1, *b1, *W2, *b2;
    const float *in_g, *in_b;
    const float *out_g, *out_b;
    const float *Wq, *qb;
    TailImages img[TAIL_IMG_MODES];
};
struct TailArgs {
    const float* A; int lda;
    const float* R; int ldr;
    const int* r_idx; const float* R2;
    const TailWeights* w;
    float* OUT; int ldo;
    float* OUT2; int ldo2;
    int M; const int* M_dev; int ff;
    bool pre;
    const TailWeights* next;
    float* QKV; int ldq; int n_qkv;
    float* scratch;
    int m_off;
    float* X1; float* H;
    float* C2; const float* ADD;
};

bool ffn_fused_supported(int ff);
int launch_ffn_fused(const float* X, int ldx, const float* W1, const float* b1, const float* W2, const float* b2,
                     const float* ln_g, const float* ln_b, float* OUT, int ldo, int M, const int* M_dev, int ff,
                     hipStream_t s);
int launch_proj_ffn_fused(const TailArgs& t, hipStream_t s);
int launch_proj_ffn_prenorm(const TailArgs& t, hipStream_t s);
bool ffn_fused_qkv_fits(int ff, int n_qkv);
#ifndef CONE_FFN_WIDE_GROUPS
#define CONE_FFN_WIDE_GROUPS 768
#endif
constexpr int FFN_WIDE_GROUPS = CONE_FFN_WIDE_GROUPS;
bool ffn_wide_supported(int ff);
int launch_proj_ffn_prenorm_wide(const TailArgs& t, hipStream_t s);
size_t ffn_spread_scratch_floats(int ff);
bool ffn_spread_supported(int M, int ff);
int launch_proj_ffn_spread(const TailArgs& t, hipStream_t s);
int launch_tail_f32_form(const TailArgs& t, int form, int n_cu, hipStream_t s);

struct TailMode {
    bool (*ffn_supported)(int ff);
    size_t (*ffn_image_bytes)(int ff);
    int (*pack)(const float* W1, const float* W2, int ff, void* img, hipStream_t s);
    int (*ffn)(const float* X, int ldx, const void* Wimg, const float* b1, const float* b2, const float* ln_g, const float* ln_b,
               float* OUT, int ldo, int M, const int* M_dev, int ff, hipStream_t s);
    bool (*rows_supported)(int N);
    size_t (*rows_image_bytes)(int N);
    int (*rows256)(const float* X, int ldx, const void* Wimg, const float* bias, float* C, int ldc, int M, const int* M_dev, int N,
                   hipStream_t s);
    size_t (*proj_image_bytes)();
    bool (*qkv_fits)(int ff, int n_qkv);
    int (*proj_ffn)(const TailArgs& t, hipStream_t s);
    int (*proj_ffn_prenorm)(const TailArgs& t, hipStream_t s);
};
extern const TailMode TAIL_MODE_SPLIT, TAIL_MODE_BF16;

int launch_layernorm(const float* x, int ldx, const float* g, const float* b, float* out, int ldo,
                     int64_t n_rows, const int* n_rows_dev, int dim, hipStream_t s, const int* src_row = nullptr);
int launch_l2norm(const float* x, int64_t n_rows, int dim, float eps, float* out, hipStream_t s, int clamp = 0);
int launch_l2norm_bf16(const float* x, int64_t n_rows, int dim, float eps, uint16_t* out, hipStream_t s, int clamp = 0);
int launch_rows_to_bf16(const float* x, int64_t n_rows, int dim, uint16_t* out, hipStream_t s);
int launch_rowdot(const float* X, int ldx, const float* W, const float* b, float* out, int ldo,
                  int64_t n_rows, int nout, int act, hipStream_t s);

enum { ATTN_PACKED = 0, ATTN_GATHER = 1, ATTN_POSADD = 2 };
struct AttnSrc {
    const float* Q; const float* K; const float* V; int ldq, ldk, ldv;
    const float* qkv_vid; const float* qkv_txt; const float* pos_qk;
    int pos_zero_row;
    const int* vrow0; const int* vlen; const int* trow0;
    const float* txt_pos_qk;
    int form;
};
int launch_enc_attn(int mode, const AttnSrc& src, float* OUT, const int* off, int B, int Lmax, hipStream_t s);
int launch_tile_rows(float* x, int period, int64_t n_rows, hipStream_t s);
int launch_tile_rows2(float* d0, const float* s0, float* d1, const float* s1, int period, int64_t n_rows, hipStream_t s);
bool dec_cross_supported(int nq, int Lmax);
int launch_dec_cross(const float* DQ, const float* XP, const float* X, const float* pos_rows, const int* vlen,
                     const int* off, const float* Wk, const float* WvT, const float* bv, float* OUT, int B, int nq,
                     int Lmax, hipStream_t s);
size_t dec_cross_mfma_slab_floats();
bool dec_cross_mfma_supported(int nq, int Lmax, bool table);
bool dec_cross_res_supported(int nq, int Lmax);
int launch_dec_cross_mfma(const float* DQ, const float* XP, const float* X, const float* pos_rows, const int* vlen,
                          const int* off, const float* Wk, const float* WvT, const float* bv, float* OUT, int B, int nq,
                          int Lmax, float* qk_slabs, hipStream_t s, int form = 2, const float* sal_w = nullptr,
                          const float* sal_b = nullptr, float* sal = nullptr, int sal_ld = 0);
int launch_small_attn(const float* Q, int ldq, const float* K, int ldk, const float* V, int ldv, float* OUT,
                      int ldo, const int* off, int B, int nq, int Lmax, hipStream_t s);

int launch_scan_lengths(const int* vlen, const int* qlen , int B, int* off, hipStream_t s);
int launch_compact_index(const int* vlen, const int* voff, int Lv_pad, int* vidx, const int* qlen, const int* toff, int Lq_pad,
                         int* tidx, int B, hipStream_t s);
int launch_pack_pos(const float* vproj, const int* vrow0, const int* vlen, const float* tproj, const int* trow0,
                    const int* qlen, const int* off, const float* dim_t, float* X, float* POS, float* XP, int B,
                    int Lmax, hipStream_t s, const float* tpe = nullptr, const float* tpg = nullptr,
                    const float* tpb = nullptr);
int launch_pos_rows(const float* dim_t, int max_v_l, float* out, hipStream_t s);
int launch_add_pos_rows(const float* MEM, const int* off, const int* vlen, const float* pos_rows, float* XP, int B, int Lmax,
                        hipStream_t s, const float* txt_pos = nullptr, const int* trow0 = nullptr);
int launch_txt_pos_rows(const float* tproj, const int* tok_index, const int* src_row, int mod, int n_emb, const float* tpe,
                        const float* tpg, const float* tpb, int n, const int* n_dev, float* out, hipStream_t s);
int launch_row_index(const int* vrow0, const int* vlen, const int* trow0, const int* qlen, const int* off, int* ridx,
                     int B, int Lmax, hipStream_t s);
int launch_pack_l0(const float* vproj, const int* vrow0, const int* vlen, const float* tproj, const int* trow0,
                   const int* qlen, const int* off, const float* dim_t, const float* qkv_vid, const float* qkv_txt,
                   const float* pos_qk, float* X, float* POS, float* QK, float* V, int B, int Lmax, hipStream_t s);
int launch_saliency(const float* MEM, const int* off, const int* vlen, const int* qlen, const float* w,
                    const float* bias, float* sal, int Lv_out, float* mem_tap, int Lq_out, int B, hipStream_t s);
int launch_proposal_mean(const float* vid, const int* vrow0, const int* vlen, const int* pad_len,
                         const float* spans, int B, int Nq, int dv, float* out, hipStream_t s);
int launch_cosine_match(const float* pf, const float* cls, const int* cls_row, int B, int Nq, int dv, float* match,
                        hipStream_t s);

bool gen_shape_supported(int d, int heads);
int launch_gen_attn(const float* Q, int ldq, const float* K, int ldk, const float* V, int ldv, float* OUT, int ldo,
                    const int* qoff, const int* koff, int B, int nq, int heads, int hd, int kcap, hipStream_t s);
int launch_gen_pack_pos(const float* vproj, const int* vrow0, const int* vlen, const float* tproj, const int* trow0,
                        const int* qlen, const int* off, const float* dim_t, float* X, float* POS, int d, int B, int Lmax,
                        hipStream_t s, const float* tpe = nullptr, const float* tpg = nullptr, const float* tpb = nullptr);
int launch_gen_pos_rows(const float* dim_t, int max_v_l, int d, float* out, hipStream_t s);
// ... 9 lines not shown
```

### cone_amd/csrc/ffn.hip

```cpp
#include <mutex>

#include "tail_f32_common.h"

namespace cone {

constexpr int FFN_STAGE = 2 * 16 * 256;
constexpr int FFN_NST = 4;

template <bool PROJ, bool QKV, int NW, bool PRE = false>
__global__ __launch_bounds__(64 * NW, NW / 4) void ffn_fused_kernel(FfnArgs p) {
    static_assert(!PRE || (PROJ && !QKV), "the pre-norm form is the layer tail");
    constexpr int FFN_ROWS = 16 * NW, FFN_NPIECE = 32 / NW, NT = 64 * NW, HW = NW / 2;
    extern __shared__ __attribute__((aligned(16))) float smem[];
    float* b1s = smem + FFN_NST * FFN_STAGE;
    TF_LAUNCH_ROWS(M, p, 0)
    const int n_tiles = (M + FFN_ROWS - 1) / FFN_ROWS;
    if (n_tiles == 0) return;
    const int G_ = (int)gridDim.x;
    const int full_items = ((n_tiles - 1) / G_) * G_;
    const int rem_rows = M - full_items * FFN_ROWS;
    const int rem_half = (rem_rows + 63) >> 6;
    const bool half_mode = NW == 8 && rem_half <= G_ && 2 * ((rem_rows + FFN_ROWS - 1) / FFN_ROWS) <= G_;
    const int n_items = full_items + (half_mode ? rem_half : (rem_rows + FFN_ROWS - 1) / FFN_ROWS);
    if ((int)blockIdx.x >= n_items) return;
    const int tid = threadIdx.x, lane = tid & 63;
    const int wave = __builtin_amdgcn_readfirstlane(tid >> 6);
    auto wave_row0 = [&](int it) -> int {
        if (it < full_items || !half_mode) return it * FFN_ROWS + wave * 16;
        return wave < 4 ? full_items * FFN_ROWS + (it - full_items) * 64 + wave * 16 : M;
    };
    const int li = lane & 15, lg = lane >> 4;
    const int ff = p.ff, nc = ff >> 4;
    constexpr int NP = PROJ ? 8 : 0;
    const int NQ = QKV ? p.n_qkv >> 5 : 0;
    const int G = NP + nc + NQ;

    float* prm = b1s + ff;
    for (int i = tid; i < (ff >> 2); i += NT)
        reinterpret_cast<f32x4*>(b1s)[i] = reinterpret_cast<const f32x4*>(p.b1)[i];
    if (tid < 64) {
        reinterpret_cast<f32x4*>(prm)[tid] = reinterpret_cast<const f32x4*>(p.b2)[tid];
        reinterpret_cast<f32x4*>(prm + 256)[tid] = reinterpret_cast<const f32x4*>(p.ln_g)[tid];
        reinterpret_cast<f32x4*>(prm + 512)[tid] = reinterpret_cast<const f32x4*>(p.ln_b)[tid];
        if (PROJ) {
            reinterpret_cast<f32x4*>(prm + 768)[tid] = reinterpret_cast<const f32x4*>(p.bo)[tid];
            reinterpret_cast<f32x4*>(prm + 1024)[tid] = reinterpret_cast<const f32x4*>(p.pg)[tid];
            reinterpret_cast<f32x4*>(prm + 1280)[tid] = reinterpret_cast<const f32x4*>(p.pb)[tid];
        }
    }
    float* qbs = prm + 1536;
    if (QKV)
        for (int i = tid; i < (p.n_qkv >> 2); i += NT)
            reinterpret_cast<f32x4*>(qbs)[i] = reinterpret_cast<const f32x4*>(p.qb)[i];

    const int drow = lane >> 2;
    const int dch = (lane & 3) ^ tf_swz16(drow);
    const bool w2side = wave >= HW;
    const float* fbase = w2side ? p.W2 : p.W1;
    const int foff = w2side ? (16 * FFN_NPIECE * (wave - HW) + drow) * ff + 4 * dch
                            : drow * 256 + 16 * FFN_NPIECE * wave + 4 * dch;
    const int fpiece = w2side ? 16 * ff : 16;
    const int fchunk = w2side ? 16 : 16 * 256;
    const int poff = PROJ ? (16 * (wave / HW) + drow) * 256 + 16 * FFN_NPIECE * (wave % HW) + 4 * dch : 0;
    int sb = 0;
    auto stream_piece = [&](int g, int i) {
        float* dstp = smem + ((sb + g) % FFN_NST) * FFN_STAGE + (wave * FFN_NPIECE + i) * 256;
        const int gg = g < G ? g : g - G;
        const bool qk = QKV && gg >= NP + nc;
        const bool pj = (PROJ && gg < NP) || qk;
        const char* ub = reinterpret_cast<const char*>(
            qk ? p.Wq + ((size_t)(gg - NP - nc) * (32 * 256) + 16 * i)
               : (pj ? p.Wo + ((size_t)gg * (32 * 256) + 16 * i) : fbase + ((size_t)(gg - NP) * fchunk + (size_t)i * fpiece)));
        const unsigned vo = (unsigned)((pj ? poff : foff) * 4);
        asm volatile("" : "+s"(ub));
        TF_GLDS16(ub + vo, dstp);
    };

    const int rd = li * 16 + ((lg ^ tf_swz16(li)) << 2);
#define FFN_RD(stg, off) (*reinterpret_cast<const f32x4*>((stg) + (off) + rd))
#define FFN_STAGE_OF(g) (smem + ((sb + (g)) % FFN_NST) * FFN_STAGE)
#define FFN_SB() __builtin_amdgcn_sched_barrier(0)
#define FFN_STREAM(g, u) { if (FFN_NPIECE == 8) stream_piece(g, u); else if ((u) & 1) stream_piece(g, (u) >> 1); }
#define FFN_END_CHUNK()                                                           \
    {                                                                             \
        FFN_SB();                                                                 \
        asm volatile("s_waitcnt vmcnt(%0)" ::"n"(FFN_NPIECE) : "memory");         \
        __builtin_amdgcn_s_barrier();                                             \
        FFN_SB();                                                                 \
    }
#define FFN_MFMA(acc, a, b) { acc = __builtin_amdgcn_mfma_f32_16x16x4f32(a, b, acc, 0, 0, 0); FFN_SB(); }
#define FFN_MM_A(acc, w0, w1, B, q)                                                   \
    {                                                                                 \
        _Pragma("unroll") for (int r = 0; r < 4; ++r) FFN_MFMA(acc[r], w0[r], B[q][r])         \
        _Pragma("unroll") for (int r = 0; r < 4; ++r) FFN_MFMA(acc[r], w1[r], B[(q) + 1][r])   \
    }
#define FFN_MM_Y(w0, w1, hh, t)                                                       \
    {                                                                                 \
        _Pragma("unroll") for (int r = 0; r < 4; ++r) {                               \
            FFN_MFMA(y[t], w0[r], hh[r])                                              \
            FFN_MFMA(y[(t) + 1], w1[r], hh[r])                                        \
        }                                                                             \
    }
#define FFN_MM_AY(acc, w0, w1, B, q, v0, v1, hh, t)                                   \
    {                                                                                 \
        _Pragma("unroll") for (int r = 0; r < 4; ++r) {                               \
            FFN_MFMA(acc[r], w0[r], B[q][r])                                          \
            FFN_MFMA(y[(t) + (r & 1)], ((r & 1) ? v1 : v0)[r >> 1], hh[r >> 1])       \
        }                                                                             \
        _Pragma("unroll") for (int r = 0; r < 4; ++r) {                               \
            FFN_MFMA(acc[r], w1[r], B[(q) + 1][r])                                    \
            FFN_MFMA(y[(t) + (r & 1)], ((r & 1) ? v1 : v0)[2 + (r >> 1)], hh[2 + (r >> 1)]) \
        }                                                                             \
    }

#define FFN_CHUNK32(gi, B)                                                                                                 \
    const float* st = FFN_STAGE_OF(gi);                                                                                    \
    f32x4 ha[2], hb[2];                                                                                                    \
    ha[0] = f32x4{0.f, 0.f, 0.f, 0.f}; hb[0] = ha[0];                                                                      \
    ha[1] = ha[0]; hb[1] = ha[0];                                                                                          \
    wa = FFN_RD(st, 0); wb = FFN_RD(st, 256); va = FFN_RD(st, 4096); vb = FFN_RD(st, 4096 + 256);                          \
    _Pragma("unroll") for (int u = 0; u < 8; ++u) {                                                                        \
        FFN_SB();                                                                                                          \
        asm volatile("" : "+v"(wa), "+v"(wb), "+v"(va), "+v"(vb));                                                         \
        FFN_SB();                                                                                                          \
        if (u < 7) {                                                                                                       \
            na = FFN_RD(st, (2 * u + 2) * 256); nb = FFN_RD(st, (2 * u + 3) * 256);                                        \
            nva = FFN_RD(st, 4096 + (2 * u + 2) * 256); nvb = FFN_RD(st, 4096 + (2 * u + 3) * 256);                        \
        }                                                                                                                  \
        FFN_SB();                                                                                                          \
        _Pragma("unroll") for (int r = 0; r < 4; ++r) {                                                                    \
            FFN_MFMA(ha[r & 1], wa[r], B[2 * u][r])                                                                        \
            FFN_MFMA(hb[r & 1], va[r], B[2 * u][r])                                                                        \
        }                                                                                                                  \
        _Pragma("unroll") for (int r = 0; r < 4; ++r) {                                                                    \
            FFN_MFMA(ha[r & 1], wb[r], B[2 * u + 1][r])                                                                    \
            FFN_MFMA(hb[r & 1], vb[r], B[2 * u + 1][r])                                                                    \
        }                                                                                                                  \
        FFN_STREAM((gi) + 2, u)                                     \
        if (u < 7) { wa = na; wb = nb; va = nva; vb = nvb; }                                                               \
    }

#pragma unroll
    for (int i = 0; i < FFN_NPIECE; ++i) stream_piece(0, i);
#pragma unroll
    for (int i = 0; i < FFN_NPIECE; ++i) stream_piece(1 < G ? 1 : 0, i);

    f32x4 wa, wb, na, nb;
    f32x4 va, vb, nva, nvb;

    f32x4 xr[16];
    f32x4 ar[PROJ ? 16 : 1];
    auto load_tile = [&](int tile) {
        const int row = wave_row0(tile) + li;
        const size_t ld_row = TF_LD_ROW(row, M);
        if (PROJ) {
            const float* ap = p.A + ld_row * p.lda + 4 * lg;
#pragma unroll
// ... 126 lines not shown
        FFN_END_CHUNK()
    }
    {
        const float* st = FFN_STAGE_OF(NP + nc - 1);
#pragma unroll
        for (int u = 0; u < 8; ++u) {
            FFN_SB();
            asm volatile("" : "+v"(va), "+v"(vb));
            FFN_SB();
            if (u < 7) { nva = FFN_RD(st, 4096 + (2 * u + 2) * 256); nvb = FFN_RD(st, 4096 + (2 * u + 3) * 256); }
            FFN_SB();
            FFN_MM_Y(va, vb, h, 2 * u)
            if (u < 7) { va = nva; vb = nvb; }
        }
    }
    FFN_SB();
    if (!PRE) {
#pragma unroll
        for (int t = 0; t < 16; ++t) y[t] = y[t] + *reinterpret_cast<const f32x4*>(prm + 16 * t + 4 * lg) + xr[t];
    }
    FFN_SB();
    load_tile(tile + (int)gridDim.x < n_items ? tile + (int)gridDim.x : tile);
    FFN_SB();
    if (PRE && my_row < M) {
        float* op = p.OUT + (size_t)my_row * p.ldo + 4 * lg;
#pragma unroll
        for (int t = 0; t < 16; ++t) *reinterpret_cast<f32x4*>(op + 16 * t) = y[t];
    }
    float rstd;
    if (!PRE || p.OUT2) tf_layernorm_regs(y, rstd);
    if (PRE) {
        if (p.OUT2 && my_row < M) {
            float* op = p.OUT2 + (size_t)my_row * p.ldo2 + 4 * lg;
            TF_LN_STORE(op, y, rstd, prm + 256, prm + 512, true, false)
        }
    } else if (my_row < M) {
        float* op = p.OUT + (size_t)my_row * p.ldo + 4 * lg;
        TF_LN_STORE(op, y, rstd, prm + 256, prm + 512, true, QKV)
    } else if (QKV) {
#pragma unroll
        for (int t = 0; t < 16; ++t) y[t] = f32x4{0.f, 0.f, 0.f, 0.f};
    }
    if (QKV) {
        float* qrow = p.QKV + (size_t)my_row * p.ldq + 4 * lg;
        for (int g = 0; g < NQ; ++g) {
            FFN_CHUNK32(NP + nc + g, y)
            FFN_SB();
            if (my_row < M) {
                *reinterpret_cast<f32x4*>(qrow + 32 * g) = (ha[0] + ha[1]) + *reinterpret_cast<const f32x4*>(qbs + 32 * g + 4 * lg);
                *reinterpret_cast<f32x4*>(qrow + 32 * g + 16) = (hb[0] + hb[1]) + *reinterpret_cast<const f32x4*>(qbs + 32 * g + 16 + 4 * lg);
            }
            FFN_END_CHUNK()
        }
    }
    sb = (sb + G) % FFN_NST;
    }
    asm volatile("s_waitcnt vmcnt(0)" ::: "memory");
}

#undef FFN_CHUNK32
#undef FFN_MM_A
#undef FFN_MM_Y
#undef FFN_MM_AY
#undef FFN_MFMA
#undef FFN_END_CHUNK
#undef FFN_SB
#undef FFN_STREAM
#undef FFN_STAGE_OF
#undef FFN_RD

bool ffn_fused_supported(int ff) { return ff >= 32 && ff % 16 == 0 && ff <= 4096; }

bool ffn_fused_qkv_fits(int ff, int n_qkv) {
    return ffn_fused_supported(ff) && n_qkv >= 32 && n_qkv % 32 == 0 &&
           (size_t)(FFN_NST * FFN_STAGE + ff + 6 * 256 + n_qkv) * sizeof(float) <= 160 * 1024;
}

static int ffn_cu_count(int* n_cu) {
    static DeviceOnce once;
    CONE_CHECK_HIP(device_once(once, [] { return hipSuccess; }, n_cu));
    return 0;
}

template <bool PROJ, bool QKV, int NW, bool PRE = false>
static int launch_ffn_nw(const TailF32Args& a, int n_cu, hipStream_t s) {
    const size_t lds = (size_t)(FFN_NST * FFN_STAGE + a.ff + 6 * 256 + (QKV ? a.n_qkv : 0)) * sizeof(float);
    CONE_REQUIRE(lds <= 160 * 1024, "fused layer tail: %zu bytes of LDS (ff %d, q|k|v %d) exceed 160 KiB", lds, a.ff, a.n_qkv);
    static DeviceOnce once;
    int dev_cu = 0;
    CONE_CHECK_HIP(device_once(once, [] {
        return hipFuncSetAttribute((const void*)ffn_fused_kernel<PROJ, QKV, NW, PRE>, hipFuncAttributeMaxDynamicSharedMemorySize,
                                   160 * 1024);
    }, &dev_cu));
    if (!n_cu) n_cu = dev_cu;
    const int tiles = (a.M + 16 * NW - 1) / (16 * NW);
    const int grid = tiles < n_cu ? tiles : n_cu;
    ProfScope ps(NW == 8 ? (PROJ ? PK_FFN_PROJ : PK_FFN_FUSED) : (PROJ ? PK_FFN_PROJ_NW4 : PK_FFN_FUSED_NW4), a.M,
                 a.ff + (QKV ? a.n_qkv / 2 : 0), 256, a.M_dev, s);
    FfnArgs k;
    static_cast<TailF32Args&>(k) = a;
    hipLaunchKernelGGL((ffn_fused_kernel<PROJ, QKV, NW, PRE>), dim3((unsigned)grid), dim3(64 * NW), lds, s, k);
    CONE_LAUNCH_CHECK();
    return 0;
}

static int launch_ffn_rows(const TailF32Args& a, bool proj, bool pre, int nw, int n_cu, hipStream_t s) {
    if (pre) return launch_ffn_nw<true, false, 8, true>(a, n_cu, s);
    if (a.Wq) return launch_ffn_nw<true, true, 8>(a, n_cu, s);
    if (nw == 4) return proj ? launch_ffn_nw<true, false, 4>(a, n_cu, s) : launch_ffn_nw<false, false, 4>(a, n_cu, s);
    return proj ? launch_ffn_nw<true, false, 8>(a, n_cu, s) : launch_ffn_nw<false, false, 8>(a, n_cu, s);
}

#ifndef CONE_FFN_SPLIT_GROUPS
#define CONE_FFN_SPLIT_GROUPS 512
#endif
static int ffn_full_round_rows(int M, int n_cu, int ff) {
    const int tiles = (M + 127) / 128;
    if (tiles <= n_cu || !ffn_wide_supported(ff)) return M;
    const int64_t full = (int64_t)(tiles / n_cu) * n_cu * 128;
    const int64_t rem = M - full;
    return rem > 0 && (rem + 15) / 16 <= CONE_FFN_SPLIT_GROUPS ? (int)full : M;
}

static int launch_ffn_ladder(TailF32Args a, bool proj, int n_cu, int wide_groups, hipStream_t s) {
    const int M = a.M;
    const bool ride = a.Wq != nullptr;
    if (!ride && (M + 15) / 16 <= wide_groups && ffn_wide_supported(a.ff)) return launch_tail_f32_wide(a, proj, false, s);
    if (!n_cu)
        if (int rc = ffn_cu_count(&n_cu)) return rc;
    const int m1 = ride ? M : ffn_full_round_rows(M, n_cu, a.ff);
    a.M = m1;
    if (int rc = launch_ffn_rows(a, proj, false, !ride && 2 * ((m1 + 127) / 128) <= n_cu ? 4 : 8, n_cu, s)) return rc;
    if (m1 == M) return 0;
    a.M = M - m1; a.m_off = m1; a.OUT += (size_t)m1 * a.ldo;
    if (!proj) a.X += (size_t)m1 * a.ldx;
    else {
        a.A += (size_t)m1 * a.lda;
        if (a.r_idx) a.r_idx += m1; else a.R += (size_t)m1 * a.ldr;
    }
    return launch_tail_f32_wide(a, proj, false, s);
}

int launch_ffn_fused(const float* X, int ldx, const float* W1, const float* b1, const float* W2, const float* b2,
                     const float* ln_g, const float* ln_b, float* OUT, int ldo, int M, const int* M_dev, int ff,
                     hipStream_t s) {
    CONE_REQUIRE(ffn_fused_supported(ff), "fused FFN: dim_feedforward=%d unsupported", ff);
    CONE_REQUIRE(X && W1 && b1 && W2 && b2 && ln_g && ln_b && OUT, "fused FFN: null argument");
    CONE_REQUIRE(ldx % 4 == 0 && ldo % 4 == 0, "fused FFN: row strides must be multiples of 4");
    if (M <= 0) return 0;
    TailF32Args a{};
    a.X = X; a.ldx = ldx; a.W1 = W1; a.b1 = b1; a.W2 = W2; a.b2 = b2; a.ln_g = ln_g; a.ln_b = ln_b;
    a.OUT = OUT; a.ldo = ldo; a.M = M; a.M_dev = M_dev; a.ff = ff;
    return launch_ffn_ladder(a, false, 0, FFN_WIDE_GROUPS, s);
}

int launch_proj_ffn_fused(const TailArgs& t, hipStream_t s) {
    if (int rc = tail_f32_check(t, TF_FORM_ROWS, "fused layer tail")) return rc;
    if (t.M <= 0) return 0;
    return launch_ffn_ladder(tail_f32_args(t), true, 0, FFN_WIDE_GROUPS, s);
}

int launch_proj_ffn_prenorm(const TailArgs& t, hipStream_t s) {
    if (int rc = tail_f32_check(t, TF_FORM_ROWS, "pre-norm layer tail")) return rc;
    if (t.M <= 0) return 0;
    return launch_ffn_rows(tail_f32_args(t), true, true, 8, 0, s);
}

int launch_tail_f32_form(const TailArgs& t, int form, int n_cu, hipStream_t s) {
    if (form == CONE_TAIL_FORM_SPREAD) return launch_proj_ffn_spread(t, s);
    CONE_REQUIRE(form >= CONE_TAIL_FORM_ROWS128 && form <= CONE_TAIL_FORM_LADDER, "tail form hook: unknown form %d", form);
    CONE_REQUIRE(!t.pre || (form != CONE_TAIL_FORM_ROWS64 && form != CONE_TAIL_FORM_LADDER), "tail form hook: no such pre-norm form");
    CONE_REQUIRE(form != CONE_TAIL_FORM_LADDER || n_cu > 0, "tail form hook: the ladder needs a CU count");
    if (int rc = tail_f32_check(t, form == CONE_TAIL_FORM_WIDE ? TF_FORM_WIDE : TF_FORM_ROWS, "tail form hook")) return rc;
    if (t.M <= 0) return 0;
    const TailF32Args a = tail_f32_args(t);
    if (form == CONE_TAIL_FORM_WIDE) return launch_tail_f32_wide(a, true, t.pre, s);
    if (form == CONE_TAIL_FORM_LADDER) return launch_ffn_ladder(a, true, n_cu, 0, s);
    return launch_ffn_rows(a, true, t.pre, form == CONE_TAIL_FORM_ROWS64 ? 4 : 8, 0, s);
}
}
```

### cone_amd/csrc/gemm_tall.hip

```cpp
#include "gemm_tall.h"
#include "tail_f32_common.h"

namespace cone {

constexpr int GT_ROWS = 128;
constexpr int GT_STAGE = 32 * 256;
constexpr int GT_NST = 4;
constexpr int GT_NPIECE = 4;
static_assert(GT_NPIECE * 8 * 256 == GT_STAGE, "8 waves x GT_NPIECE pieces of 256 floats fill a stage");
static_assert(GT_NST == 4, "the stage index is advanced with & 3, and chunk c + 2 must not land in a stage still being read");

template <bool RES>
__global__ __launch_bounds__(512, 2) void gemm_tall_kernel(GemmArgs p) {
    extern __shared__ __attribute__((aligned(16))) float smem[];
    float* bs = smem + GT_NST * GT_STAGE;
    int M = p.M;
    if (p.M_dev) { const int md = *p.M_dev; M = md < M ? md : M; }
    const int n_tiles = M > 0 ? (M + GT_ROWS - 1) / GT_ROWS : 0;
    if ((int)blockIdx.x >= n_tiles) return;
    const int tid = threadIdx.x, lane = tid & 63;
    const int wave = __builtin_amdgcn_readfirstlane(tid >> 6);
    const int li = lane & 15, lg = lane >> 4;
    const int NC = p.N >> 5;
    const bool relu = (p.flags & EPI_RELU) != 0;

    for (int i = tid; i < (p.N >> 2); i += 512)
        reinterpret_cast<f32x4*>(bs)[i] = p.bias ? reinterpret_cast<const f32x4*>(p.bias)[i] : f32x4{0.f, 0.f, 0.f, 0.f};

    const int drow = lane >> 2;
    const int dch = (lane & 3) ^ tf_swz16(drow);
    const unsigned vo = (unsigned)(((16 * (wave >> 2) + drow) * 256 + 16 * GT_NPIECE * (wave & 3) + 4 * dch) * 4);
    int stg = 0;
    int ws = 0;
    auto stream_piece = [&](int stage, int wchunk, int i) {
        float* dstp = smem + stage * GT_STAGE + (wave * GT_NPIECE + i) * 256;
        const char* ub = reinterpret_cast<const char*>(p.W + ((size_t)wchunk * (32 * 256) + 16 * i));
        asm volatile("" : "+s"(ub));
        TF_GLDS16(ub + vo, dstp);
    };
    auto next_chunk = [&]() { ws = ws + 1 < NC ? ws + 1 : 0; stg = (stg + 1) & 3; };

    const int rd = li * 16 + ((lg ^ tf_swz16(li)) << 2);
#define GT_RD(stp, off) (*reinterpret_cast<const f32x4*>((stp) + (off) + rd))
#define GT_SB() __builtin_amdgcn_sched_barrier(0)
#define GT_END_CHUNK()                                                            \
    {                                                                             \
        GT_SB();                                                                  \
        asm volatile("s_waitcnt vmcnt(%0)" ::"n"(GT_NPIECE) : "memory");          \
        __builtin_amdgcn_s_barrier();                                             \
        GT_SB();                                                                  \
    }
#define GT_MFMA(acc, a, b) { acc = __builtin_amdgcn_mfma_f32_16x16x4f32(a, b, acc, 0, 0, 0); GT_SB(); }

    f32x4 x[16], xn[16];
    auto load_rows = [&](int tile) {
        const float* ap = p.A + TF_LD_ROW(tile * GT_ROWS + wave * 16 + li, M) * p.lda + 4 * lg;
#pragma unroll
        for (int q = 0; q < 16; ++q)
            asm volatile("global_load_dwordx4 %0, %1, off offset:%2" : "=v"(xn[q]) : "v"(ap), "n"(64 * q) : "memory");
    };
#define GT_ROWS_LANDED()                                                                                         \
    asm volatile("" : "+v"(xn[0]), "+v"(xn[1]), "+v"(xn[2]), "+v"(xn[3]), "+v"(xn[4]), "+v"(xn[5]), "+v"(xn[6]),  \
                      "+v"(xn[7]), "+v"(xn[8]), "+v"(xn[9]), "+v"(xn[10]), "+v"(xn[11]), "+v"(xn[12]),           \
                      "+v"(xn[13]), "+v"(xn[14]), "+v"(xn[15]))
    load_rows(blockIdx.x);
    {
        const int w1 = NC > 1 ? 1 : 0;
#pragma unroll
        for (int i = 0; i < GT_NPIECE; ++i) stream_piece(0, 0, i);
#pragma unroll
        for (int i = 0; i < GT_NPIECE; ++i) stream_piece(1, w1, i);
        ws = w1 + 1 < NC ? w1 + 1 : 0;
    }

    f32x4 wa, wb, na, nb;
    f32x4 va, vb, nva, nvb;
    asm volatile("s_waitcnt vmcnt(%0)" ::"n"(GT_NPIECE) : "memory");
    GT_ROWS_LANDED();
    __syncthreads();
    for (int tile = blockIdx.x; tile < n_tiles; tile += gridDim.x) {
        const int my_row0 = tile * GT_ROWS + wave * 16;
        const int my_row = my_row0 + li;
        const bool act = my_row0 < M;
        if (!act) {
            for (int g = 0; g < NC; ++g) {
#pragma unroll
                for (int i = 0; i < GT_NPIECE; ++i) stream_piece((stg + 2) & 3, ws, i);
                GT_END_CHUNK()
                next_chunk();
            }
            break;
        }
#pragma unroll
        for (int q = 0; q < 16; ++q) x[q] = xn[q];
        GT_SB();
        float* cp = p.C + (size_t)my_row * p.ldc + 4 * lg;
        const float* rp = RES ? p.R + TF_LD_ROW(my_row, M) * p.ldr + 4 * lg : nullptr;
        f32x4 r0, r1;
        if (RES) { r0 = *reinterpret_cast<const f32x4*>(rp); r1 = *reinterpret_cast<const f32x4*>(rp + 16); }
        GT_SB();

        for (int g = 0; g < NC; ++g) {
            if (g == 0) load_rows(tile + (int)gridDim.x < n_tiles ? tile + (int)gridDim.x : tile);
            const float* st = smem + stg * GT_STAGE;
            const int sn = (stg + 2) & 3;
            f32x4 ha = f32x4{0.f, 0.f, 0.f, 0.f}, hb = ha;
            wa = GT_RD(st, 0); wb = GT_RD(st, 256); va = GT_RD(st, 4096); vb = GT_RD(st, 4096 + 256);
#pragma unroll
            for (int u = 0; u < 8; ++u) {
                GT_SB();
                asm volatile("" : "+v"(wa), "+v"(wb), "+v"(va), "+v"(vb));
                GT_SB();
                if (u < 7) {
                    na = GT_RD(st, (2 * u + 2) * 256); nb = GT_RD(st, (2 * u + 3) * 256);
                    nva = GT_RD(st, 4096 + (2 * u + 2) * 256); nvb = GT_RD(st, 4096 + (2 * u + 3) * 256);
                }
                GT_SB();
#pragma unroll
                for (int r = 0; r < 4; ++r) {
                    GT_MFMA(ha, wa[r], x[2 * u][r])
                    GT_MFMA(hb, va[r], x[2 * u][r])
                }
#pragma unroll
                for (int r = 0; r < 4; ++r) {
                    GT_MFMA(ha, wb[r], x[2 * u + 1][r])
                    GT_MFMA(hb, vb[r], x[2 * u + 1][r])
                }
                if (u & 1) stream_piece(sn, ws, u >> 1);
                if (u < 7) { wa = na; wb = nb; va = nva; vb = nvb; }
            }
            GT_SB();
            f32x4 o0 = ha + *reinterpret_cast<const f32x4*>(bs + 32 * g + 4 * lg);
            f32x4 o1 = hb + *reinterpret_cast<const f32x4*>(bs + 32 * g + 16 + 4 * lg);
            if (relu) {
#pragma unroll
                for (int r = 0; r < 4; ++r) { o0[r] = fmaxf(o0[r], 0.f); o1[r] = fmaxf(o1[r], 0.f); }
            }
            if (RES) { o0 += r0; o1 += r1; }
            asm volatile("" : "+v"(o0), "+v"(o1));
            GT_END_CHUNK()
            GT_ROWS_LANDED();
            if (my_row < M) {
                *reinterpret_cast<f32x4*>(cp + 32 * g) = o0;
                *reinterpret_cast<f32x4*>(cp + 32 * g + 16) = o1;
            }
            if (RES) {
                const int gn = g + 1 < NC ? g + 1 : g;
                r0 = *reinterpret_cast<const f32x4*>(rp + 32 * gn);
                r1 = *reinterpret_cast<const f32x4*>(rp + 32 * gn + 16);
            }
            GT_SB();
            next_chunk();
        }
    }
    asm volatile("s_waitcnt vmcnt(0)" ::: "memory");
}

#undef GT_ROWS_LANDED
#undef GT_MFMA
#undef GT_END_CHUNK
#undef GT_SB
#undef GT_RD

static size_t gt_lds_bytes(int N) { return (size_t)(GT_NST * GT_STAGE + N) * sizeof(float); }

const char* gemm_tall_refusal(const GemmArgs& a) {
    if (a.K != 256) return "K must be 256";
    if (a.N < 32 || a.N % 32 != 0 || gt_lds_bytes(a.N) > 160 * 1024) return "N must be a multiple of 32 up to 8192";
    if (a.ldw != 256) return "the weight rows must be contiguous (ldw == 256)";
    if (a.A2) return "no fused addend (A2)";
    if (a.C2 || a.ADD) return "no second output (C2 / ADD)";
    if (a.flags & EPI_LN) return "no LayerNorm epilogue";
    if (a.r_mod) return "no row-periodic residual (r_mod)";
    if (a.m_off) return "no row offset (m_off)";
    if (a.lda % 4 != 0 || a.ldc % 4 != 0 || ((a.flags & EPI_RESIDUAL) && a.ldr % 4 != 0)) return "row strides must be multiples of 4";
    return nullptr;
}

int launch_gemm_tall(const GemmArgs& a, int n_cu, hipStream_t s) {
    const char* why = gemm_tall_refusal(a);
    CONE_REQUIRE(!why, "gemm: the tall form (variant %d) cannot run this launch: %s (M=%d N=%d K=%d flags=%d)", GEMM_TALL, why,
                 a.M, a.N, a.K, a.flags);
    CONE_REQUIRE(a.A && a.W && a.C && (!(a.flags & EPI_RESIDUAL) || a.R), "gemm: the tall form: null argument");
    if (a.M <= 0) return 0;
    static DeviceOnce once;
    int dev_cu = 0;
    CONE_CHECK_HIP(device_once(once, [] {
        hipError_t rc = hipFuncSetAttribute((const void*)gemm_tall_kernel<false>, hipFuncAttributeMaxDynamicSharedMemorySize, 160 * 1024);
        if (rc == hipSuccess)
            rc = hipFuncSetAttribute((const void*)gemm_tall_kernel<true>, hipFuncAttributeMaxDynamicSharedMemorySize, 160 * 1024);
        return rc;
    }, &dev_cu));
    if (n_cu <= 0) n_cu = dev_cu;
    const int tiles = (a.M + GT_ROWS - 1) / GT_ROWS;
    const int grid = tiles < n_cu ? tiles : n_cu;
    ProfScope ps(PK_GEMM_ROWS16, a.M, a.N, a.K, a.M_dev, s);
    if (a.flags & EPI_RESIDUAL)
        hipLaunchKernelGGL(gemm_tall_kernel<true>, dim3((unsigned)grid), dim3(512), gt_lds_bytes(a.N), s, a);
    else
        hipLaunchKernelGGL(gemm_tall_kernel<false>, dim3((unsigned)grid), dim3(512), gt_lds_bytes(a.N), s, a);
    CONE_LAUNCH_CHECK();
    return 0;
}

}
```

### cone_amd/csrc/tail_f32_common.h

```cpp
#pragma once

#include "common.h"

namespace cone {

#define TF_GLDS16(src, dst) \
    __builtin_amdgcn_global_load_lds((const __attribute__((address_space(1))) void*)(src), \
                                     (__attribute__((address_space(3))) void*)(dst), 16, 0, 0)

__device__ __forceinline__ int tf_swz16(int row) { return (0x1230 >> (((row >> 2) & 3) * 4)) & 3; }

__device__ __forceinline__ void tf_layernorm_regs(f32x4 (&v)[16], float& rstd) {
    float s1 = 0.f;
#pragma unroll
    for (int t = 0; t < 16; ++t) s1 += (v[t][0] + v[t][1]) + (v[t][2] + v[t][3]);
    s1 += __shfl_xor(s1, 16, 64);
    s1 += __shfl_xor(s1, 32, 64);
    const float mean = s1 * (1.0f / 256.0f);
    float s2 = 0.f;
#pragma unroll
    for (int t = 0; t < 16; ++t) {
#pragma unroll
        for (int r = 0; r < 4; ++r) { v[t][r] -= mean; s2 = fmaf(v[t][r], v[t][r], s2); }
    }
    s2 += __shfl_xor(s2, 16, 64);
    s2 += __shfl_xor(s2, 32, 64);
    rstd = 1.0f / sqrtf(s2 * (1.0f / 256.0f) + 1e-5f);
}
#define TF_LN_TILE(o, v, rstd, gp, bp, t)                                                       \
    {                                                                                           \
        const f32x4 g_ = *reinterpret_cast<const f32x4*>((gp) + 16 * (t) + 4 * lg);             \
        const f32x4 b_ = *reinterpret_cast<const f32x4*>((bp) + 16 * (t) + 4 * lg);             \
        _Pragma("unroll") for (int r = 0; r < 4; ++r) o[r] = v[t][r] * rstd * g_[r] + b_[r];    \
    }
#define TF_LN_APPLY(v, rstd, gp, bp) \
    _Pragma("unroll") for (int t = 0; t < 16; ++t) TF_LN_TILE(v[t], v, rstd, gp, bp, t)
#define TF_LN_STORE(op, v, rstd, gp, bp, WHEN, KEEP)             \
    _Pragma("unroll") for (int t = 0; t < 16; ++t) {             \
        if (WHEN) {                                              \
            f32x4 o_;                                            \
            TF_LN_TILE(o_, v, rstd, gp, bp, t)                   \
            *reinterpret_cast<f32x4*>((op) + 16 * t) = o_;       \
            if (KEEP) v[t] = o_;                                 \
        }                                                        \
    }

#define TF_LAUNCH_ROWS(M, p, m_off) \
    int M = (p).M;                  \
    if ((p).M_dev) { const int md_ = *(p).M_dev - (m_off); M = md_ < M ? md_ : M; }
#define TF_LD_ROW(row, M) ((size_t)((row) < (M) ? (row) : (M) - 1))
#define TF_RES_ROW(rp, p, ld_row, off)                                                                               \
    const float* rp = (p).R + (ld_row) * (p).ldr + (off);                                                            \
    if ((p).r_idx) {                                                                                                 \
        const int ix_ = (p).r_idx[ld_row];                                                                           \
        rp = (ix_ >= 0 ? (p).R + (size_t)ix_ * (p).ldr : (p).R2 + (size_t)(~ix_) * (p).ldr) + (off);                 \
    }

struct TailF32Args {
    const float* X; int ldx;
    const float* W1; const float* b1;
    const float* W2; const float* b2;
    const float* ln_g; const float* ln_b;
    float* OUT; int ldo;
    int M; const int* M_dev;
    int ff;
    const float* A; int lda; const float* R; int ldr;
    const float* Wo; const float* bo; const float* pg; const float* pb;
    const int* r_idx; const float* R2;
    const float* Wq; const float* qb; float* QKV; int ldq; int n_qkv;
    float* OUT2; int ldo2;
    int m_off;
};
struct FfnArgs : TailF32Args {};
struct FfnWideArgs : TailF32Args {};

enum { TF_FORM_ROWS = 0, TF_FORM_WIDE = 1, TF_FORM_SPREAD = 2 };

bool ffn_fused_supported(int ff);
bool ffn_wide_supported(int ff);
bool ffn_spread_supported(int M, int ff);

static inline bool tail_f32_rides(const TailArgs& t) { return !t.pre && t.next && t.next->Wq; }

static inline TailF32Args tail_f32_args(const TailArgs& t) {
    const TailWeights& w = *t.w;
    TailF32Args a{};
    a.A = t.A; a.lda = t.lda; a.Wo = w.Wo; a.bo = w.bo; a.R = t.R; a.ldr = t.ldr; a.pg = w.in_g; a.pb = w.in_b;
    a.r_idx = t.r_idx; a.R2 = t.R2;
    a.W1 = w.W1; a.b1 = w.b1; a.W2 = w.W2; a.b2 = w.b2;
    a.ln_g = t.pre && !w.out_g ? w.in_g : w.out_g; a.ln_b = t.pre && !w.out_b ? w.in_b : w.out_b;
    a.OUT = t.OUT; a.ldo = t.ldo; a.M = t.M; a.M_dev = t.M_dev; a.ff = t.ff; a.m_off = t.m_off;
    if (t.pre) { a.OUT2 = t.OUT2; a.ldo2 = t.ldo2; }
    if (tail_f32_rides(t)) { a.Wq = t.next->Wq; a.qb = t.next->qb; a.QKV = t.QKV; a.ldq = t.ldq; a.n_qkv = t.n_qkv; }
    return a;
}

static inline int tail_f32_check(const TailArgs& t, int form, const char* what) {
    const TailWeights& w = *t.w;
    CONE_REQUIRE(form != TF_FORM_SPREAD || (ffn_spread_supported(t.M, t.ff) && t.scratch), "%s: unsupported size M=%d ff=%d", what,
                 t.M, t.ff);
    CONE_REQUIRE(!t.r_idx || t.R2, "%s: a gathered residual needs both source matrices", what);
    CONE_REQUIRE(form == TF_FORM_SPREAD || (form == TF_FORM_WIDE ? ffn_wide_supported(t.ff) : ffn_fused_supported(t.ff)),
                 "%s: dim_feedforward=%d unsupported", what, t.ff);
    CONE_REQUIRE(t.A && w.Wo && w.bo && t.R && w.in_g && w.in_b && w.W1 && w.b1 && w.W2 && w.b2 && t.OUT &&
                     (t.pre ? !t.OUT2 || (w.out_g && w.out_b) : w.out_g && w.out_b), "%s: null argument", what);
    CONE_REQUIRE(t.lda % 4 == 0 && t.ldr % 4 == 0 && t.ldo % 4 == 0 && (!t.pre || !t.OUT2 || t.ldo2 % 4 == 0),
                 "%s: row strides must be multiples of 4", what);
    CONE_REQUIRE(form != TF_FORM_ROWS || !tail_f32_rides(t) ||
                     (t.next->qb && t.QKV && t.n_qkv >= 32 && t.n_qkv % 32 == 0 && t.ldq % 4 == 0), "%s: bad q|k|v arguments", what);
    return 0;
}

int launch_tail_f32_wide(const TailF32Args& a, bool proj, bool pre, hipStream_t s);
int launch_tail_f32_spread(const TailF32Args& a, bool pre, float* scratch, hipStream_t s);

}
```

### include/cone_hip.h

```cpp
#ifndef CONE_HIP_H
#define CONE_HIP_H

#include <stddef.h>
#include <stdint.h>

#ifdef __cplusplus
extern "C" {
#endif

#define CONE_HIP_ABI_VERSION 8

#define CONE_E_INVALID (-1)
#define CONE_E_HIP (-2)
#define CONE_E_WORKSPACE (-3)

#define CONE_MAX_LAYERS 8
#define CONE_MAX_PROJ 3
#define CONE_TABLE_MAX_V_L 255
#define CONE_MAX_WINDOW_TOKENS 256
#define CONE_MAX_LONG_WINDOW_TOKENS 1024

typedef struct cone_model cone_model;

typedef struct { const float* w; const float* b; } cone_linear_w;
// ... 276 lines not shown

size_t cone_library_localize_ragged_workspace(const cone_model* m, const cone_library* lib, const int32_t* q_row0,
                                              const int32_t* q_ctx_l, const int32_t* tok_len, int nq, const int32_t* pair_k,
                                              const cone_session_params* params, int ranked);
int cone_library_localize_ragged(const cone_model* m, const cone_library* lib, const int32_t* q_row0, const int32_t* q_ctx_l,
                                 const float* tok, const int32_t* tok_len, int nq, const float* cls, const int32_t* pair_k,
                                 const cone_session_params* params, const int32_t* pair_query, const int32_t* pair_slot,
                                 const int32_t* scan_widx, const float* scan_wval, int scan_nq, int64_t scan_n_videos, int scan_K,
                                 double* kept, int32_t* n_kept, void* ws, size_t ws_bytes, void* stream);


int cone_corpus_fuse_nms(const float* cand, const int32_t* seg_off, const int64_t* seg_cand, const int32_t* seg_n,
                         const int32_t* seg_tag, int nq, int n_seg, double nms_thd, int max_before, int max_after,
                         double* out_rows, int32_t* out_seg, int32_t* out_n, void* stream);

size_t cone_library_localize_candidates_workspace(const cone_model* m, const cone_library* lib, const int32_t* q_row0,
                                                  const int32_t* q_ctx_l, const int32_t* tok_len, int nq, const int32_t* pair_k,
                                                  const cone_session_params* params, int ranked);
int cone_library_localize_candidates(const cone_model* m, const cone_library* lib, const int32_t* q_row0, const int32_t* q_ctx_l,
                                     const float* tok, const int32_t* tok_len, int nq, const float* cls, const int32_t* pair_k,
                                     const cone_session_params* params, const int32_t* pair_query, const int32_t* pair_slot,
                                     const int32_t* scan_widx, const float* scan_wval, int scan_nq, int64_t scan_n_videos, int scan_K,
                                     float* cand, void* ws, size_t ws_bytes, void* stream);


int cone_watch_plan(const int32_t* widx, const float* wval, int nq, int K, const int32_t* stamp, int n_win, int ctx_l, int W, int Nq,
                    int32_t* miss_widx, float* miss_wval, int32_t* n_miss, int32_t* seg_off, int64_t* seg_cand,
                    int32_t* seg_n, int32_t* seg_tag, void* stream);

int cone_watch_store(const float* cand, const int32_t* miss_widx, const int32_t* n_miss, int nq, int K, int n_win, int ctx_l, int Nq,
                     float* cache, int32_t* stamp, void* stream);


int cone_watch_pool_plan(const int32_t* widx, const float* wval, const int32_t* n_pairs, const int32_t* pair_slot,
                         const int32_t* pair_k, const int32_t* v_ctx_l, const int32_t* v_win0, const int32_t* v_cap,
                         const int32_t* stamp, int nq, int V, int K, int Wb, int n_win_total, int W, int Nq, int32_t* miss_widx,
                         float* miss_wval, int32_t* pair_miss, int32_t* seg_off, int64_t* seg_cand, int32_t* seg_n,
                         int32_t* seg_tag, void* stream);

int cone_watch_pool_store(const float* cand, const int32_t* jobs, int n_jobs, const int32_t* miss_widx, const int32_t* v_ctx_l,
                          const int32_t* v_win0, const int32_t* v_cap, int nq, int V, int K, int n_win_total, int Nq, float* cache,
                          int32_t* stamp, void* stream);


typedef struct {
    const cone_model* model;
    int64_t capacity;
    int32_t v_dim;
    uint16_t* rows_bf16;
    float* err;
} cone_library_shadow;

size_t cone_library_shadow_bytes(const cone_library* lib);
int cone_library_shadow_open(const cone_library* lib, void* arena, size_t arena_bytes, cone_library_shadow* out);

int cone_library_shadow_index(const cone_model* m, const cone_library* lib, const cone_library_shadow* shadow, int64_t row0,
                              int64_t n_rows, void* stream);

size_t cone_library_scan_certified_workspace(const cone_library* lib, int64_t n_videos, int64_t total_hb, int64_t total_win, int nq,
                                             int K, int W, int n_cand);
int cone_library_scan_certified(const cone_model* m, const cone_library* lib, const cone_library_shadow* shadow,
                                const int64_t* v_row0, const int32_t* v_ctx_l, const int64_t* v_hb_off, const int64_t* v_win_off,
                                int64_t n_videos, int64_t total_hb, int64_t total_win, const float* cls, int nq, int K, int W,
                                int n_cand, const cone_session_params* params, int32_t* widx, float* wval, int32_t* certified,
                                void* ws, size_t ws_bytes, void* stream);

int cone_eval_recall(const double* rows, const int32_t* n, const double* gt, int nq, int max_after,
                     const double* thresholds, int n_thr, const int32_t* topk, int n_topk, int mode,
                     int64_t* hits, double* top1_iou, void* stream);
int cone_eval_window_recall(const int32_t* win_idx, int nq, int k, const double* gt, double clip_length,
                            int slide, const int32_t* topk, int n_topk, int64_t* hits, void* stream);

int cone_prof_enable(int on);
int64_t cone_prof_collect(double* out, int64_t max_rec);

int cone_model_set_option(cone_model* m, const char* name, int value);
int cone_test_gemm(const float* A, const float* A2, int a2_mod, const float* W, const float* bias,
                   const float* R, const float* ln_g, const float* ln_b, float* C, float* C2,
                   const float* ADD, int M, int N, int K, int flags, void* stream);
int cone_test_gemm_tall(const float* A, const float* A2, int a2_mod, const float* W, const float* bias,
                        const float* R, const float* ln_g, const float* ln_b, float* C, float* C2,
                        const float* ADD, int M, int N, int K, int flags, int lda, int ldc, const int32_t* M_dev,
                        int n_cu, void* stream);
size_t cone_test_gemm_bf16_image_bytes(int N, int K);
int cone_test_gemm_bf16(const float* A, const float* A2, int a2_mod, const float* W, const float* bias,
                        const float* R, const float* ln_g, const float* ln_b, float* C, float* C2,
                        const float* ADD, int M, int N, int K, int flags, void* img, int ldc, int r_mod,
                        const int32_t* M_dev, void* stream);
int cone_test_ffn(const float* X, const float* W1, const float* b1, const float* W2, const float* b2,
                  const float* ln_g, const float* ln_b, float* OUT, int M, int ff, void* stream);
int cone_test_proj_ffn(const float* A, const float* Wo, const float* bo, const float* R, const float* pg, const float* pb,
                       const float* W1, const float* b1, const float* W2, const float* b2, const float* ln_g,
                       const float* ln_b, float* OUT, int M, int ff, void* stream);
#define CONE_TEST_PACK 1
#define CONE_TEST_SINGLE_PIECE 2
size_t cone_test_ffn_split_image_bytes(int ff);
int cone_test_ffn_split(const float* X, const float* W1, const float* b1, const float* W2, const float* b2,
                        const float* ln_g, const float* ln_b, float* OUT, int M, int ff, void* img, int pack, void* stream);
size_t cone_test_rows_split_image_bytes(int N);
int cone_test_rows_split(const float* X, const float* W, const float* bias, float* C, int M, int N, void* img, int pack,
                         void* stream);
#define CONE_FFN_SPREAD_MAX_ROWS 1024
size_t cone_test_proj_ffn_spread_scratch_bytes(int ff);
int cone_test_proj_ffn_spread(const float* A, const float* Wo, const float* bo, const float* R, const float* pg, const float* pb,
                              const float* W1, const float* b1, const float* W2, const float* b2, const float* ln_g,
                              const float* ln_b, float* OUT, int M, int ff, void* scratch, void* stream);
enum { CONE_TAIL_FORM_ROWS128 = 0, CONE_TAIL_FORM_ROWS64 = 1, CONE_TAIL_FORM_WIDE = 2, CONE_TAIL_FORM_LADDER = 3,
       CONE_TAIL_FORM_SPREAD = 4 };
int cone_test_tail_form(const float* A, const float* Wo, const float* bo, const float* R, const float* pg, const float* pb,
                        const float* W1, const float* b1, const float* W2, const float* b2, const float* ln_g,
                        const float* ln_b, float* OUT, int M, int ff, const int32_t* r_idx, const float* R2,
                        const int32_t* M_dev, int pre, float* OUT2, int form, int n_cu, void* scratch, void* stream);
size_t cone_test_proj_split_image_bytes(void);
int cone_test_proj_ffn_split(const float* A, const float* Wo, const float* bo, const float* R, const float* pg,
                             const float* pb, const float* W1, const float* b1, const float* W2, const float* b2,
                             const float* ln_g, const float* ln_b, float* OUT, int M, int ff, void* img, void* wo_img,
                             int pack, void* stream);
int cone_test_enc_attn(int mode, const float* QKV, const float* qkv_vid, const float* qkv_txt, const float* pos_qk,
                       const int32_t* vrow0, const int32_t* vlen, const int32_t* trow0, const int32_t* off, float* OUT,
                       int B, int Lmax, int pos_zero_row , void* stream);
int cone_test_dec_cross(const float* DQ, const float* X, const float* pos_rows, const int32_t* vlen, const int32_t* off,
                        const float* Wk, const float* WvT, const float* bv, float* OUT, int B, int nq, int Lmax,
                        int variant, float* qk_slabs, void* stream);
size_t cone_test_dec_cross_slab_floats(void);
int cone_test_enc_attn_txt(int mode, const float* QKV, const float* qkv_vid, const float* qkv_txt, const float* pos_qk,
                           const float* txt_pos_qk, const int32_t* vrow0, const int32_t* vlen, const int32_t* trow0,
                           const int32_t* off, float* OUT, int B, int Lmax, int pos_zero_row, void* stream);
int cone_test_small_attn(const float* Q, int ldq, const float* K, int ldk, const float* V, int ldv, float* OUT, int ldo,
                         const int32_t* off, int B, int nq, int Lmax, void* stream);
int cone_test_dec_cross_ex(const float* DQ, const float* XP, const float* X, const float* pos_rows, const int32_t* vlen,
                           const int32_t* off, const float* Wk, const float* WvT, const float* bv, float* OUT, int B, int nq,
                           int Lmax, int variant, float* qk_slabs, const float* sal_w, const float* sal_b, float* sal,
                           int sal_ld, void* stream);
int cone_test_layernorm(const float* x, const float* g, const float* b, float* out, int64_t n_rows,
                        int dim, void* stream);
int cone_test_gen_attn(const float* Q, int ldq, const float* K, int ldk, const float* V, int ldv, float* OUT, int ldo,
                       const int32_t* qoff, const int32_t* koff, int B, int nq, int heads, int head_dim, int kcap, void* stream);

int cone_test_grid_limit_y(void);
int cone_test_scan_lengths(const int32_t* vlen, const int32_t* qlen, int B, int32_t* off, void* stream);
int cone_test_compact_index(const int32_t* vlen, const int32_t* voff, int Lv_pad, int32_t* vidx, const int32_t* qlen,
                            const int32_t* toff, int Lq_pad, int32_t* tidx, int B, void* stream);
int cone_test_pack_pos(const float* vproj, const int32_t* vrow0, const int32_t* vlen, const float* tproj, const int32_t* trow0,
                       const int32_t* qlen, const int32_t* off, const float* dim_t, float* X, float* POS, float* XP, int B,
                       int Lmax, const float* tpe, const float* tpg, const float* tpb, void* stream);
int cone_test_gen_pack_pos(const float* vproj, const int32_t* vrow0, const int32_t* vlen, const float* tproj,
                           const int32_t* trow0, const int32_t* qlen, const int32_t* off, const float* dim_t, float* X, float* POS,
                           int d, int B, int Lmax, const float* tpe, const float* tpg, const float* tpb, void* stream);
int cone_test_pack_l0(const float* vproj, const int32_t* vrow0, const int32_t* vlen, const float* tproj, const int32_t* trow0,
                      const int32_t* qlen, const int32_t* off, const float* dim_t, const float* qkv_vid, const float* qkv_txt,
                      const float* pos_qk, float* X, float* POS, float* QK, float* V, int B, int Lmax, void* stream);
int cone_test_row_index(const int32_t* vrow0, const int32_t* vlen, const int32_t* trow0, const int32_t* qlen, const int32_t* off,
                        int32_t* ridx, int B, int Lmax, void* stream);
int cone_test_add_pos_rows(const float* MEM, const int32_t* off, const int32_t* vlen, const float* pos_rows, float* XP, int B,
                           int Lmax, const float* txt_pos, const int32_t* trow0, void* stream);
int cone_test_txt_pos_rows(const float* tproj, const int32_t* tok_index, const int32_t* src_row, int mod, int n_emb,
                           const float* tpe, const float* tpg, const float* tpb, int n, const int32_t* n_dev, float* out,
                           void* stream);
int cone_test_gen_txt_pos_rows(const float* tproj, const int32_t* tok_index, const int32_t* src_row, int mod, int n_emb,
                               const float* tpe, const float* tpg, const float* tpb, int n, const int32_t* n_dev, int d,
                               float* out, void* stream);
int cone_test_saliency(const float* MEM, const int32_t* off, const int32_t* vlen, const int32_t* qlen, const float* w,
                       const float* bias, float* sal, int Lv_out, float* mem_tap, int Lq_out, int B, void* stream);
int cone_test_gen_saliency(const float* MEM, const int32_t* off, const int32_t* vlen, const int32_t* qlen, const float* w,
                           const float* bias, float* sal, int Lv_out, float* mem_tap, int Lq_out, int B, int d, void* stream);
int cone_test_rowdot(const float* X, int ldx, const float* W, const float* b, float* out, int ldo, int64_t n_rows, int nout,
// ... 11 lines not shown
```

Before: 375,700.

## Pre-pack fp32 tail and tall-GEMM weights into contiguous per-lane stream images

```diff
diff --git a/cone_amd/_lib.py b/cone_amd/_lib.py
--- a/cone_amd/_lib.py
+++ b/cone_amd/_lib.py
@@ -246,6 +246,14 @@
     "cone_test_gemm_tall": (C.c_int, [C.c_void_p, C.c_void_p, C.c_int, C.c_void_p, C.c_void_p, C.c_void_p,
                                       C.c_void_p, C.c_void_p, C.c_void_p, C.c_void_p, C.c_void_p, C.c_int, C.c_int,
                                       C.c_int, C.c_int, C.c_int, C.c_int, C.c_void_p, C.c_int, C.c_void_p]),
+    "cone_test_f32_pack_tail_bytes": (C.c_size_t, [C.c_int, C.c_int, C.c_int]),
+    "cone_test_f32_pack_tail": (C.c_int, [C.c_void_p] * 3 + [C.c_int, C.c_void_p, C.c_int, C.c_void_p, C.c_void_p]),
+    "cone_test_f32_pack_rows_bytes": (C.c_size_t, [C.c_int]),
+    "cone_test_f32_packed_launches": (C.c_long, [C.c_int]),
+    "cone_test_f32_pack_rows": (C.c_int, [C.c_void_p, C.c_int, C.c_void_p, C.c_void_p]),
+    "cone_test_gemm_tall_packed": (C.c_int, [C.c_void_p] * 5 + [C.c_int] * 3 + [C.c_void_p, C.c_int, C.c_void_p, C.c_void_p]),
+    "cone_test_tail_packed": (C.c_int, [C.c_void_p] * 13 + [C.c_int] * 3 + [C.c_void_p] * 4 + [C.c_int] * 3
+                              + [C.c_void_p, C.c_void_p]),
     "cone_test_gemm_bf16_image_bytes": (C.c_size_t, [C.c_int, C.c_int]),
     "cone_test_gemm_bf16": (C.c_int, [C.c_void_p, C.c_void_p, C.c_int, C.c_void_p, C.c_void_p, C.c_void_p,
                                       C.c_void_p, C.c_void_p, C.c_void_p, C.c_void_p, C.c_void_p, C.c_int, C.c_int,
diff --git a/cone_amd/build.py b/cone_amd/build.py
--- a/cone_amd/build.py
+++ b/cone_amd/build.py
@@ -12,7 +12,7 @@
 PYLISTS = os.path.join(HERE, "_cone_pylists.so")
 SOURCES = ["api.hip", "gemm.hip", "rowops.hip", "attention.hip", "window_ops.hip", "prefilter.hip",
            "postproc.hip", "prof.hip", "dec_cross.hip", "metrics.hip", "ffn.hip", "criterion.hip", "dec_cross_mfma.hip", "ffn_split.hip", "ffn_wide.hip",
-           "general.hip", "ffn_bf16.hip", "gemm_bf16.hip", "gemm_tall.hip", "session.hip", "library_move.hip",
+           "general.hip", "ffn_bf16.hip", "gemm_bf16.hip", "gemm_tall.hip", "tail_pack.hip", "session.hip", "library_move.hip",
            "library_budget.hip", "library_corpus.hip", "library_watch.hip", "library_watch_pool.hip"]
 FLAGS = ["-O3", "--offload-arch=gfx950", "-fPIC", "-std=c++17", "-Wall", "-Wno-unused-function"]
 NO_CONTRACT = {"window_ops.hip", "postproc.hip", "metrics.hip", "criterion.hip", "general.hip", "library_corpus.hip"}
diff --git a/cone_amd/csrc/api.hip b/cone_amd/csrc/api.hip
--- a/cone_amd/csrc/api.hip
+++ b/cone_amd/csrc/api.hip
@@ -65,6 +65,20 @@
     struct GenImage { const float* W; const void* img; };
     std::vector<GenImage> gen_bf16_images;
     int opt_max_tokens = CONE_MAX_WINDOW_TOKENS;
+    char* f32_img = nullptr; char* f32_tall_img = nullptr;
+    struct TallImage { const float* W; int N; const char* img; };
+    std::vector<TallImage> tall_images;
+    int opt_tail_packed = CONE_TAIL_PACKED_DEFAULT;
+    int opt_gemm_tall_packed = CONE_GEMM_TALL_PACKED_DEFAULT;
+    const void* tall_image(const float* W, int N) const {
+        for (const TallImage& t : tall_images) {
+            const uintptr_t w = (uintptr_t)W, base = (uintptr_t)t.W;
+            if (w < base || (w - base) % (32 * 256 * sizeof(float)) != 0) continue;
+            const size_t off = (w - base) / sizeof(float);
+            if (off / 256 + (size_t)N <= (size_t)t.N) return t.img + (size_t)(off / (32 * 256)) * cone::F32_PACK_CHUNK_BYTES;
+        }
+        return nullptr;
+    }
     bool long_windows() const { return opt_max_tokens > CONE_MAX_WINDOW_TOKENS; }
     bool general() const { return gen_native || opt_general || long_windows(); }
 };
@@ -90,6 +104,8 @@
     if (m->split_img) (void)hipFree(m->split_img);
     if (m->bf16_img) (void)hipFree(m->bf16_img);
     if (m->gen_bf16_img) (void)hipFree(m->gen_bf16_img);
+    if (m->f32_img) (void)hipFree(m->f32_img);
+    if (m->f32_tall_img) (void)hipFree(m->f32_tall_img);
     if (m->tab_arena) (void)hipFree(m->tab_arena);
     delete m;
 }
@@ -113,6 +129,48 @@
         if (int rc = k.pack(t.W1, t.W2, m->ff, ip + k.proj_image_bytes(), nullptr)) return rc;
         t.img[mode].wo = ip; t.img[mode].ffn = ip + k.proj_image_bytes();
     }
+    return 0;
+}
+
+static int build_f32_images(cone_model* m) {
+    const int ff = m->ff, nl = m->n_enc + m->n_dec;
+    size_t total = 0;
+    for (int i = 0; i < nl; ++i) total += f32_pack_tail_bytes(ff, true, i + 1 < m->n_enc ? 768 : 0);
+    if (hipMalloc((void**)&m->f32_img, total) != hipSuccess) {
+        set_error("model_create: hipMalloc of %zu bytes of packed fp32 weight streams failed", total);
+        return CONE_E_HIP;
+    }
+    char* ip = m->f32_img;
+    for (int i = 0; i < nl; ++i) {
+        TailWeights& t = i < m->n_enc ? m->enc_tail[i] : m->dec_tail[i - m->n_enc];
+        const float* Wq = i + 1 < m->n_enc ? m->enc_tail[i + 1].Wq : nullptr;
+        if (int rc = launch_f32_pack_tail(t.Wo, t.W1, t.W2, ff, Wq, 768, ip, nullptr)) return rc;
+        t.pk = ip; t.pk_nq = Wq ? 768 : 0;
+        ip += f32_pack_tail_bytes(ff, true, t.pk_nq);
+    }
+    return 0;
+}
+static int build_tall_images(cone_model* m) {
+    if (m->f32_tall_img) return 0;
+    const int nl = m->n_enc + m->n_dec;
+    if (hipMalloc((void**)&m->f32_tall_img, (size_t)nl * f32_pack_rows_bytes(768)) != hipSuccess) {
+        set_error("gemm_tall_packed: hipMalloc of %zu bytes of packed fp32 weight streams failed", (size_t)nl * f32_pack_rows_bytes(768));
+        return CONE_E_HIP;
+    }
+    char* ip = m->f32_tall_img;
+    std::vector<cone_model::TallImage> images;
+    int rc = 0;
+    for (int i = 0; i < nl && rc == 0; ++i, ip += f32_pack_rows_bytes(768)) {
+        const float* W = i < m->n_enc ? m->enc[i].sa.in_w : m->dec[i - m->n_enc].sa.in_w;
+        rc = launch_f32_pack_rows(W, 768, ip, nullptr);
+        images.push_back({W, 768, ip});
+    }
+    if (rc == 0 && hipDeviceSynchronize() != hipSuccess) {
+        set_error("gemm_tall_packed: building the weight images failed");
+        rc = CONE_E_HIP;
+    }
+    if (rc) { (void)hipFree(m->f32_tall_img); m->f32_tall_img = nullptr; return rc; }
+    m->tall_images.swap(images);
     return 0;
 }
 
@@ -296,6 +354,12 @@
             return CONE_E_HIP;
         }
     }
+    if (!m->gen_native && ffn_fused_supported(m->ff)) {
+        if (build_f32_images(m) != 0 || hipDeviceSynchronize() != hipSuccess || (m->opt_gemm_tall_packed && build_tall_images(m) != 0)) {
+            free_model(m);
+            return CONE_E_HIP;
+        }
+    }
     if (dec0_constants(m, nullptr) != 0 || hipDeviceSynchronize() != hipSuccess) {
         free_model(m);
         return CONE_E_HIP;
@@ -336,6 +400,7 @@
     g.M = M; g.M_dev = M_dev; g.N = N; g.K = K; g.flags = flags;
     g.variant = m ? m->opt_gemm | ((m->opt_gemm_tall_min + 1) << GEMM_TALL_MIN_SHIFT) : GEMM_AUTO;
     if (m && !m->opt_spread) g.flags |= GEMM_NO_SPREAD;
+    if (m && m->opt_gemm_tall_packed && K == 256 && ldw == 256) g.Wimg = m->tall_image(W, N);
     return g;
 }
 
@@ -689,6 +754,7 @@
     const bool spread = m->opt_spread && f.SPR && ffn_spread_supported(t.M, ff);
     t.next = nullptr;
     t.scratch = f.SPR;
+    t.packed = m->opt_tail_packed != 0;
     *rode = false;
     if (t.pre) {
         if (bf16) return TAIL_MODES[TAIL_IMG_BF16]->proj_ffn_prenorm(t, s);
@@ -1350,6 +1416,7 @@
     {"rows_chain", &cone_model::opt_chain, 0, 1, true},
     {"ffn_spread", &cone_model::opt_spread, 0, 1, true},
     {"gemm_tall_min_rows", &cone_model::opt_gemm_tall_min, -1, GEMM_TALL_MIN_MAX, false},
+    {"tail_packed", &cone_model::opt_tail_packed, 0, 1, true},
 };
 extern "C" int cone_model_set_option(cone_model* m, const char* name, int value) {
     CONE_REQUIRE(m && name, "set_option: null argument");
@@ -1394,6 +1461,12 @@
         m->opt_general_bf16 = 1;
         return 0;
     }
+    if (!strcmp(name, "gemm_tall_packed")) {
+        if (value != 0 && !m->gen_native)
+            if (int rc = build_tall_images(m)) return rc;
+        m->opt_gemm_tall_packed = value != 0;
+        return 0;
+    }
     if (!strcmp(name, "gemm")) {
         CONE_REQUIRE(value >= GEMM_AUTO && value <= GEMM_TALL, "set_option: gemm tile family %d not in [0, 4]", value);
         m->opt_gemm = value;
@@ -1433,6 +1506,23 @@
     CONE_REQUIRE(n_cu >= 0, "gemm tall hook: negative CU count");
     return n_cu > 0 ? launch_gemm_tall(g, n_cu, (hipStream_t)stream) : launch_gemm(g, (hipStream_t)stream);
 }
+extern "C" size_t cone_test_f32_pack_tail_bytes(int ff, int proj, int n_qkv) { return f32_pack_tail_bytes(ff, proj != 0, n_qkv); }
+extern "C" int cone_test_f32_pack_tail(const float* Wo, const float* W1, const float* W2, int ff, const float* Wq, int n_qkv,
+                                       void* img, void* stream) {
+    return launch_f32_pack_tail(Wo, W1, W2, ff, Wq, n_qkv, img, (hipStream_t)stream);
+}
+extern "C" long cone_test_f32_packed_launches(int which) { return f32_packed_launches(which); }
+extern "C" size_t cone_test_f32_pack_rows_bytes(int N) { return f32_pack_rows_bytes(N); }
+extern "C" int cone_test_f32_pack_rows(const float* W, int N, void* img, void* stream) {
+    return launch_f32_pack_rows(W, N, img, (hipStream_t)stream);
+}
+extern "C" int cone_test_gemm_tall_packed(const float* A, const float* W, const float* bias, const float* R, float* C, int M,
+                                          int N, int flags, const int32_t* M_dev, int n_cu, const void* img, void* stream) {
+    GemmArgs g = G(nullptr, A, 256, W, 256, bias, C, N, M, M_dev, N, 256, flags & (EPI_RELU | EPI_RESIDUAL));
+    g.variant = GEMM_TALL; g.R = R; g.ldr = N; g.Wimg = img;
+    CONE_REQUIRE(n_cu >= 0, "gemm tall hook: negative CU count");
+    return launch_gemm_tall(g, n_cu, (hipStream_t)stream);
+}
 extern "C" size_t cone_test_gemm_bf16_image_bytes(int N, int K) { return gemm_bf16_image_bytes(N, K); }
 extern "C" int cone_test_gemm_bf16(const float* A, const float* A2, int a2_mod, const float* W, const float* bias,
                                    const float* R, const float* ln_g, const float* ln_b, float* C, float* C2,
@@ -1480,6 +1570,17 @@
     TailArgs t = test_tail(&w, A, Wo, bo, R, pg, pb, W1, b1, W2, b2, ln_g, ln_b, OUT, M, ff);
     t.r_idx = r_idx; t.R2 = R2; t.M_dev = M_dev; t.pre = pre != 0; t.OUT2 = OUT2; t.ldo2 = 256; t.scratch = (float*)scratch;
     return launch_tail_f32_form(t, form, n_cu, (hipStream_t)stream);
+}
+extern "C" int cone_test_tail_packed(const float* A, const float* Wo, const float* bo, const float* R, const float* pg,
+                                     const float* pb, const float* W1, const float* b1, const float* W2, const float* b2,
+                                     const float* ln_g, const float* ln_b, float* OUT, int M, int ff, int pre, float* OUT2,
+                                     const float* Wq, const float* qb, float* QKV, int n_qkv, int nw, int n_cu, const void* img,
+                                     void* stream) {
+    TailWeights w, nx{};
+    TailArgs t = test_tail(&w, A, Wo, bo, R, pg, pb, W1, b1, W2, b2, ln_g, ln_b, OUT, M, ff);
+    t.pre = pre != 0; t.OUT2 = OUT2; t.ldo2 = 256;
+    if (Wq) { nx.Wq = Wq; nx.qb = qb; t.next = &nx; t.QKV = QKV; t.ldq = n_qkv; t.n_qkv = n_qkv; }
+    return launch_tail_f32_rows_hook(t, img, nw, n_cu, (hipStream_t)stream);
 }
 static int test_tail_mode(int pack, bool* do_pack) {
     const bool single = pack & CONE_TEST_SINGLE_PIECE;
diff --git a/cone_amd/csrc/common.h b/cone_amd/csrc/common.h
--- a/cone_amd/csrc/common.h
+++ b/cone_amd/csrc/common.h
@@ -107,6 +107,7 @@
     int N, K;
     int flags;
     int variant;
+    const void* Wimg;
 };
 enum { GEMM_AUTO = 0, GEMM_SQUARE = 1, GEMM_ROWS4 = 2, GEMM_ROWS8 = 3 };
 int launch_gemm(const GemmArgs& a, hipStream_t s);
@@ -124,6 +125,7 @@
     const float *out_g, *out_b;
     const float *Wq, *qb;
     TailImages img[TAIL_IMG_MODES];
+    const void* pk; int pk_nq;
 };
 struct TailArgs {
     const float* A; int lda;
@@ -140,6 +142,7 @@
     int m_off;
     float* X1; float* H;
     float* C2; const float* ADD;
+    bool packed;
 };
 
 bool ffn_fused_supported(int ff);
@@ -159,6 +162,22 @@
 bool ffn_spread_supported(int M, int ff);
 int launch_proj_ffn_spread(const TailArgs& t, hipStream_t s);
 int launch_tail_f32_form(const TailArgs& t, int form, int n_cu, hipStream_t s);
+
+constexpr size_t F32_PACK_CHUNK_BYTES = 32 * 1024;
+#ifndef CONE_TAIL_PACKED_DEFAULT
+#define CONE_TAIL_PACKED_DEFAULT 1
+#endif
+#ifndef CONE_GEMM_TALL_PACKED_DEFAULT
+#define CONE_GEMM_TALL_PACKED_DEFAULT 0
+#endif
+size_t f32_pack_tail_bytes(int ff, bool proj, int n_qkv);
+int launch_f32_pack_tail(const float* Wo, const float* W1, const float* W2, int ff, const float* Wq, int n_qkv, void* img,
+                         hipStream_t s);
+size_t f32_pack_rows_bytes(int N);
+int launch_f32_pack_rows(const float* W, int N, void* img, hipStream_t s);
+void f32_packed_note(int which);
+long f32_packed_launches(int which);
+int launch_tail_f32_rows_hook(const TailArgs& t, const void* img, int nw, int n_cu, hipStream_t s);
 
 struct TailMode {
     bool (*ffn_supported)(int ff);
diff --git a/cone_amd/csrc/ffn.hip b/cone_amd/csrc/ffn.hip
--- a/cone_amd/csrc/ffn.hip
+++ b/cone_amd/csrc/ffn.hip
@@ -7,7 +7,7 @@
 constexpr int FFN_STAGE = 2 * 16 * 256;
 constexpr int FFN_NST = 4;
 
-template <bool PROJ, bool QKV, int NW, bool PRE = false>
+template <bool PROJ, bool QKV, int NW, bool PRE = false, bool PK = false>
 __global__ __launch_bounds__(64 * NW, NW / 4) void ffn_fused_kernel(FfnArgs p) {
     static_assert(!PRE || (PROJ && !QKV), "the pre-norm form is the layer tail");
     constexpr int FFN_ROWS = 16 * NW, FFN_NPIECE = 32 / NW, NT = 64 * NW, HW = NW / 2;
@@ -63,16 +63,26 @@
     const int fchunk = w2side ? 16 : 16 * 256;
     const int poff = PROJ ? (16 * (wave / HW) + drow) * 256 + 16 * FFN_NPIECE * (wave % HW) + 4 * dch : 0;
     int sb = 0;
+    unsigned pkvo = (unsigned)(lane * 16);
+    unsigned poff4 = (unsigned)(poff * 4), foff4 = (unsigned)(foff * 4);
     auto stream_piece = [&](int g, int i) {
         float* dstp = smem + ((sb + g) % FFN_NST) * FFN_STAGE + (wave * FFN_NPIECE + i) * 256;
         const int gg = g < G ? g : g - G;
+        if (PK) {
+            const char* ub = reinterpret_cast<const char*>(p.Wimg) + (((unsigned)gg << 15) + (unsigned)(wave * FFN_NPIECE + i) * 1024u);
+            asm volatile("" : "+s"(ub));
+            asm volatile("" : "+v"(pkvo));
+            TF_GLDS16(ub + pkvo, dstp);
+            return;
+        }
         const bool qk = QKV && gg >= NP + nc;
         const bool pj = (PROJ && gg < NP) || qk;
         const char* ub = reinterpret_cast<const char*>(
             qk ? p.Wq + ((size_t)(gg - NP - nc) * (32 * 256) + 16 * i)
                : (pj ? p.Wo + ((size_t)gg * (32 * 256) + 16 * i) : fbase + ((size_t)(gg - NP) * fchunk + (size_t)i * fpiece)));
-        const unsigned vo = (unsigned)((pj ? poff : foff) * 4);
         asm volatile("" : "+s"(ub));
+        asm volatile("" : "+v"(poff4), "+v"(foff4));
+        const unsigned vo = pj ? poff4 : foff4;
         TF_GLDS16(ub + vo, dstp);
     };
 
@@ -365,14 +375,14 @@
     return 0;
 }
 
-template <bool PROJ, bool QKV, int NW, bool PRE = false>
+template <bool PROJ, bool QKV, int NW, bool PRE = false, bool PK = false>
 static int launch_ffn_nw(const TailF32Args& a, int n_cu, hipStream_t s) {
     const size_t lds = (size_t)(FFN_NST * FFN_STAGE + a.ff + 6 * 256 + (QKV ? a.n_qkv : 0)) * sizeof(float);
     CONE_REQUIRE(lds <= 160 * 1024, "fused layer tail: %zu bytes of LDS (ff %d, q|k|v %d) exceed 160 KiB", lds, a.ff, a.n_qkv);
     static DeviceOnce once;
     int dev_cu = 0;
     CONE_CHECK_HIP(device_once(once, [] {
-        return hipFuncSetAttribute((const void*)ffn_fused_kernel<PROJ, QKV, NW, PRE>, hipFuncAttributeMaxDynamicSharedMemorySize,
+        return hipFuncSetAttribute((const void*)ffn_fused_kernel<PROJ, QKV, NW, PRE, PK>, hipFuncAttributeMaxDynamicSharedMemorySize,
                                    160 * 1024);
     }, &dev_cu));
     if (!n_cu) n_cu = dev_cu;
@@ -382,16 +392,21 @@
                  a.ff + (QKV ? a.n_qkv / 2 : 0), 256, a.M_dev, s);
     FfnArgs k;
     static_cast<TailF32Args&>(k) = a;
-    hipLaunchKernelGGL((ffn_fused_kernel<PROJ, QKV, NW, PRE>), dim3((unsigned)grid), dim3(64 * NW), lds, s, k);
+    hipLaunchKernelGGL((ffn_fused_kernel<PROJ, QKV, NW, PRE, PK>), dim3((unsigned)grid), dim3(64 * NW), lds, s, k);
     CONE_LAUNCH_CHECK();
+    if (PK) f32_packed_note(0);
     return 0;
 }
 
+template <bool PK>
+static int launch_ffn_rows_pk(const TailF32Args& a, bool proj, bool pre, int nw, int n_cu, hipStream_t s) {
+    if (pre) return launch_ffn_nw<true, false, 8, true, PK>(a, n_cu, s);
+    if (a.Wq) return launch_ffn_nw<true, true, 8, false, PK>(a, n_cu, s);
+    if (nw == 4) return proj ? launch_ffn_nw<true, false, 4, false, PK>(a, n_cu, s) : launch_ffn_nw<false, false, 4, false, PK>(a, n_cu, s);
+    return proj ? launch_ffn_nw<true, false, 8, false, PK>(a, n_cu, s) : launch_ffn_nw<false, false, 8, false, PK>(a, n_cu, s);
+}
 static int launch_ffn_rows(const TailF32Args& a, bool proj, bool pre, int nw, int n_cu, hipStream_t s) {
-    if (pre) return launch_ffn_nw<true, false, 8, true>(a, n_cu, s);
-    if (a.Wq) return launch_ffn_nw<true, true, 8>(a, n_cu, s);
-    if (nw == 4) return proj ? launch_ffn_nw<true, false, 4>(a, n_cu, s) : launch_ffn_nw<false, false, 4>(a, n_cu, s);
-    return proj ? launch_ffn_nw<true, false, 8>(a, n_cu, s) : launch_ffn_nw<false, false, 8>(a, n_cu, s);
+    return a.Wimg ? launch_ffn_rows_pk<true>(a, proj, pre, nw, n_cu, s) : launch_ffn_rows_pk<false>(a, proj, pre, nw, n_cu, s);
 }
 
 #ifndef CONE_FFN_SPLIT_GROUPS
@@ -461,4 +476,27 @@
     if (form == CONE_TAIL_FORM_LADDER) return launch_ffn_ladder(a, true, n_cu, 0, s);
     return launch_ffn_rows(a, true, t.pre, form == CONE_TAIL_FORM_ROWS64 ? 4 : 8, 0, s);
 }
-}
+
+int launch_tail_f32_rows_hook(const TailArgs& t, const void* img, int nw, int n_cu, hipStream_t s) {
+    CONE_REQUIRE(nw == 8 || nw == 4, "tail rows hook: %d waves", nw);
+    CONE_REQUIRE(n_cu >= 0, "tail rows hook: negative CU count");
+    const bool proj = t.A != nullptr;
+    CONE_REQUIRE(proj || (!t.pre && !t.next), "tail rows hook: the block alone has no pre-norm form and no ride");
+    CONE_REQUIRE(nw == 8 || (!t.pre && !t.next), "tail rows hook: the ride and the pre-norm form run on 8 waves");
+    TailF32Args a;
+    if (proj) {
+        if (int rc = tail_f32_check(t, TF_FORM_ROWS, "tail rows hook")) return rc;
+        a = tail_f32_args(t);
+    } else {
+        const TailWeights& w = *t.w;
+        CONE_REQUIRE(ffn_fused_supported(t.ff) && t.R && w.W1 && w.b1 && w.W2 && w.b2 && w.out_g && w.out_b && t.OUT,
+                     "tail rows hook: bad block arguments");
+        a = TailF32Args{};
+        a.X = t.R; a.ldx = t.ldr; a.W1 = w.W1; a.b1 = w.b1; a.W2 = w.W2; a.b2 = w.b2; a.ln_g = w.out_g; a.ln_b = w.out_b;
+        a.OUT = t.OUT; a.ldo = t.ldo; a.M = t.M; a.M_dev = t.M_dev; a.ff = t.ff;
+    }
+    a.Wimg = img;
+    if (t.M <= 0) return 0;
+    return launch_ffn_rows(a, proj, t.pre, nw, n_cu, s);
+}
+}
diff --git a/cone_amd/csrc/gemm_tall.hip b/cone_amd/csrc/gemm_tall.hip
--- a/cone_amd/csrc/gemm_tall.hip
+++ b/cone_amd/csrc/gemm_tall.hip
@@ -10,7 +10,7 @@
 static_assert(GT_NPIECE * 8 * 256 == GT_STAGE, "8 waves x GT_NPIECE pieces of 256 floats fill a stage");
 static_assert(GT_NST == 4, "the stage index is advanced with & 3, and chunk c + 2 must not land in a stage still being read");
 
-template <bool RES>
+template <bool RES, bool PK = false>
 __global__ __launch_bounds__(512, 2) void gemm_tall_kernel(GemmArgs p) {
     extern __shared__ __attribute__((aligned(16))) float smem[];
     float* bs = smem + GT_NST * GT_STAGE;
@@ -29,13 +29,16 @@
 
     const int drow = lane >> 2;
     const int dch = (lane & 3) ^ tf_swz16(drow);
-    const unsigned vo = (unsigned)(((16 * (wave >> 2) + drow) * 256 + 16 * GT_NPIECE * (wave & 3) + 4 * dch) * 4);
+    unsigned vo = PK ? (unsigned)(lane * 16)
+                           : (unsigned)(((16 * (wave >> 2) + drow) * 256 + 16 * GT_NPIECE * (wave & 3) + 4 * dch) * 4);
     int stg = 0;
     int ws = 0;
     auto stream_piece = [&](int stage, int wchunk, int i) {
         float* dstp = smem + stage * GT_STAGE + (wave * GT_NPIECE + i) * 256;
-        const char* ub = reinterpret_cast<const char*>(p.W + ((size_t)wchunk * (32 * 256) + 16 * i));
+        const char* ub = PK ? reinterpret_cast<const char*>(p.Wimg) + (((unsigned)wchunk << 15) + (unsigned)(wave * GT_NPIECE + i) * 1024u)
+                            : reinterpret_cast<const char*>(p.W + ((size_t)wchunk * (32 * 256) + 16 * i));
         asm volatile("" : "+s"(ub));
+        asm volatile("" : "+v"(vo));
         TF_GLDS16(ub + vo, dstp);
     };
     auto next_chunk = [&]() { ws = ws + 1 < NC ? ws + 1 : 0; stg = (stg + 1) & 3; };
@@ -186,20 +189,23 @@
     static DeviceOnce once;
     int dev_cu = 0;
     CONE_CHECK_HIP(device_once(once, [] {
-        hipError_t rc = hipFuncSetAttribute((const void*)gemm_tall_kernel<false>, hipFuncAttributeMaxDynamicSharedMemorySize, 160 * 1024);
-        if (rc == hipSuccess)
-            rc = hipFuncSetAttribute((const void*)gemm_tall_kernel<true>, hipFuncAttributeMaxDynamicSharedMemorySize, 160 * 1024);
+        const void* const kernels[4] = {(const void*)gemm_tall_kernel<false, false>, (const void*)gemm_tall_kernel<true, false>,
+                                        (const void*)gemm_tall_kernel<false, true>, (const void*)gemm_tall_kernel<true, true>};
+        hipError_t rc = hipSuccess;
+        for (int i = 0; i < 4 && rc == hipSuccess; ++i)
+            rc = hipFuncSetAttribute(kernels[i], hipFuncAttributeMaxDynamicSharedMemorySize, 160 * 1024);
         return rc;
     }, &dev_cu));
     if (n_cu <= 0) n_cu = dev_cu;
     const int tiles = (a.M + GT_ROWS - 1) / GT_ROWS;
     const int grid = tiles < n_cu ? tiles : n_cu;
     ProfScope ps(PK_GEMM_ROWS16, a.M, a.N, a.K, a.M_dev, s);
-    if (a.flags & EPI_RESIDUAL)
-        hipLaunchKernelGGL(gemm_tall_kernel<true>, dim3((unsigned)grid), dim3(512), gt_lds_bytes(a.N), s, a);
-    else
-        hipLaunchKernelGGL(gemm_tall_kernel<false>, dim3((unsigned)grid), dim3(512), gt_lds_bytes(a.N), s, a);
+    const bool res = (a.flags & EPI_RESIDUAL) != 0;
+    auto* const kernel = a.Wimg ? (res ? gemm_tall_kernel<true, true> : gemm_tall_kernel<false, true>)
+                                : (res ? gemm_tall_kernel<true, false> : gemm_tall_kernel<false, false>);
+    hipLaunchKernelGGL(kernel, dim3((unsigned)grid), dim3(512), gt_lds_bytes(a.N), s, a);
     CONE_LAUNCH_CHECK();
+    if (a.Wimg) f32_packed_note(1);
     return 0;
 }
 
diff --git a/cone_amd/csrc/tail_f32_common.h b/cone_amd/csrc/tail_f32_common.h
--- a/cone_amd/csrc/tail_f32_common.h
+++ b/cone_amd/csrc/tail_f32_common.h
@@ -70,6 +70,7 @@
     const float* Wq; const float* qb; float* QKV; int ldq; int n_qkv;
     float* OUT2; int ldo2;
     int m_off;
+    const void* Wimg;
 };
 struct FfnArgs : TailF32Args {};
 struct FfnWideArgs : TailF32Args {};
@@ -92,6 +93,7 @@
     a.OUT = t.OUT; a.ldo = t.ldo; a.M = t.M; a.M_dev = t.M_dev; a.ff = t.ff; a.m_off = t.m_off;
     if (t.pre) { a.OUT2 = t.OUT2; a.ldo2 = t.ldo2; }
     if (tail_f32_rides(t)) { a.Wq = t.next->Wq; a.qb = t.next->qb; a.QKV = t.QKV; a.ldq = t.ldq; a.n_qkv = t.n_qkv; }
+    if (t.packed && w.pk && (!a.Wq || w.pk_nq == a.n_qkv)) a.Wimg = w.pk;
     return a;
 }
 
diff --git a/cone_amd/csrc/tail_pack.hip b/cone_amd/csrc/tail_pack.hip
--- /dev/null
+++ b/cone_amd/csrc/tail_pack.hip
@@ -0,0 +1,60 @@
+#include <atomic>
+
+#include "tail_f32_common.h"
+
+namespace cone {
+
+__global__ __launch_bounds__(256) void f32_pack_kernel(const float* __restrict__ Wo, const float* __restrict__ W1,
+                                                       const float* __restrict__ W2, const float* __restrict__ Wq, int np, int nf,
+                                                       int nq, int ff, f32x4* __restrict__ img, int n16) {
+    const int idx = blockIdx.x * 256 + threadIdx.x;
+    if (idx >= n16) return;
+    const int l = idx & 63, s = (idx >> 6) & 31, g = idx >> 11;
+    const int row = l >> 2, ch = (l & 3) ^ tf_swz16(row);
+    const float* src;
+    if (g < np || g >= np + nf) {
+        const float* W = g < np ? Wo : Wq;
+        const int c = g < np ? g : g - np - nf;
+        src = W + (size_t)(32 * c + 16 * (s >> 4) + row) * 256 + 16 * (s & 15) + 4 * ch;
+    } else {
+        const int c = g - np;
+        src = s < 16 ? W1 + (size_t)(16 * c + row) * 256 + 16 * s + 4 * ch
+                     : W2 + (size_t)(16 * (s - 16) + row) * ff + 16 * c + 4 * ch;
+    }
+    img[idx] = *reinterpret_cast<const f32x4*>(src);
+}
+
+static std::atomic<long> g_packed_launches[2];
+void f32_packed_note(int which) { g_packed_launches[which & 1].fetch_add(1, std::memory_order_relaxed); }
+long f32_packed_launches(int which) { return g_packed_launches[which & 1].load(std::memory_order_relaxed); }
+
+size_t f32_pack_tail_bytes(int ff, bool proj, int n_qkv) {
+    if (!ffn_fused_supported(ff) || n_qkv < 0 || n_qkv % 32 != 0) return 0;
+    return (size_t)((proj ? 8 : 0) + ff / 16 + n_qkv / 32) * F32_PACK_CHUNK_BYTES;
+}
+size_t f32_pack_rows_bytes(int N) { return N >= 32 && N % 32 == 0 ? (size_t)(N / 32) * F32_PACK_CHUNK_BYTES : 0; }
+
+static int pack_launch(const float* Wo, const float* W1, const float* W2, const float* Wq, int np, int nf, int nq, int ff,
+                       void* img, hipStream_t s) {
+    const int n16 = (np + nf + nq) * (int)(F32_PACK_CHUNK_BYTES / 16);
+    hipLaunchKernelGGL(f32_pack_kernel, dim3((unsigned)((n16 + 255) / 256)), dim3(256), 0, s, Wo, W1, W2, Wq, np, nf, nq, ff,
+                       (f32x4*)img, n16);
+    CONE_LAUNCH_CHECK();
+    return 0;
+}
+
+int launch_f32_pack_tail(const float* Wo, const float* W1, const float* W2, int ff, const float* Wq, int n_qkv, void* img,
+                         hipStream_t s) {
+    CONE_REQUIRE(ffn_fused_supported(ff), "fp32 tail image: dim_feedforward=%d unsupported", ff);
+    CONE_REQUIRE(W1 && W2 && img, "fp32 tail image: null argument");
+    CONE_REQUIRE(!Wq || (n_qkv >= 32 && n_qkv % 32 == 0 && n_qkv <= 8192), "fp32 tail image: q|k|v width %d not a multiple of 32", n_qkv);
+    return pack_launch(Wo, W1, W2, Wq, Wo ? 8 : 0, ff / 16, Wq ? n_qkv / 32 : 0, ff, img, s);
+}
+
+int launch_f32_pack_rows(const float* W, int N, void* img, hipStream_t s) {
+    CONE_REQUIRE(W && img, "fp32 row image: null argument");
+    CONE_REQUIRE(N >= 32 && N % 32 == 0 && N <= 8192, "fp32 row image: N=%d must be a multiple of 32 up to 8192", N);
+    return pack_launch(W, nullptr, nullptr, nullptr, N / 32, 0, 0, 0, img, s);
+}
+
+}
diff --git a/include/cone_hip.h b/include/cone_hip.h
--- a/include/cone_hip.h
+++ b/include/cone_hip.h
@@ -382,6 +382,18 @@
                         const float* R, const float* ln_g, const float* ln_b, float* C, float* C2,
                         const float* ADD, int M, int N, int K, int flags, int lda, int ldc, const int32_t* M_dev,
                         int n_cu, void* stream);
+size_t cone_test_f32_pack_tail_bytes(int ff, int proj, int n_qkv);
+int cone_test_f32_pack_tail(const float* Wo, const float* W1, const float* W2, int ff, const float* Wq, int n_qkv, void* img,
+                            void* stream);
+size_t cone_test_f32_pack_rows_bytes(int N);
+long cone_test_f32_packed_launches(int which);
+int cone_test_f32_pack_rows(const float* W, int N, void* img, void* stream);
+int cone_test_gemm_tall_packed(const float* A, const float* W, const float* bias, const float* R, float* C, int M, int N,
+                               int flags, const int32_t* M_dev, int n_cu, const void* img, void* stream);
+int cone_test_tail_packed(const float* A, const float* Wo, const float* bo, const float* R, const float* pg, const float* pb,
+                          const float* W1, const float* b1, const float* W2, const float* b2, const float* ln_g,
+                          const float* ln_b, float* OUT, int M, int ff, int pre, float* OUT2, const float* Wq, const float* qb,
+                          float* QKV, int n_qkv, int nw, int n_cu, const void* img, void* stream);
 size_t cone_test_gemm_bf16_image_bytes(int N, int K);
 int cone_test_gemm_bf16(const float* A, const float* A2, int a2_mod, const float* W, const float* bias,
                         const float* R, const float* ln_g, const float* ln_b, float* C, float* C2,
```

Result: faster. 381,300, median of 6 (+1.5%).
